# dayae1204/WeCLIP-ViT-CoMer

Measured on AMD Instinct MI355X. Metric: images/sec (train fwd+bwd) ViT-B/16 512x512 VOC, higher is better.
Workload: dtype f16 MFMA operands / f32 accumulate, f32 residual+softmax+LN, PAR f32 arithmetic on 16-bit fixed-point affinities (precision=fast); 1 GPU; WeCLIP VOC full train step (the reference's model: frozen CLIP ViT-B/16 + adapters + decoder + GradCAM/affinity/PAR pseudo-labels), batch 16/GPU at 512x512, K=2 classes/image (BASELINE configs[2] without the ViT-CoMer inserts, for which the reference has no code); global_batch=16, parallelism=dp1

## Files before the change

### include/weclip_hip.h

```cpp
#ifndef WECLIP_HIP_H
#define WECLIP_HIP_H
#include <stdint.h>
#ifdef __cplusplus
extern "C" {
#endif

int wc_version(void);
const char* wc_last_error(void);
int wc_device_count(void);
int wc_device_arch(int dev, char* buf, int buflen);

void wc_prof_enable(int stride);
void wc_prof_tag(const char* tag);
int wc_prof_report(char* buf, int cap);

int wc_par_affinity(const float* img, float* aff, int B, int H, int W,
                    const int* h_dilations, int n_dil, void* stream);
int wc_par_iterate(const float* aff, const float* masks_in, float* masks_out, int B, int C,
                   int H, int W, const int* h_dilations, int n_dil, void* stream);
int wc_par_forward(const float* img, const float* masks, float* out, float* tmp, float* aff_ws,
                   int B, int C, int H, int W, const int* h_dilations, int n_dil, int num_iter,
                   int group, void* stream);
int wc_par_forward_h(const float* img, const float* masks, float* out, float* tmp, float* aff_ws,
                   int B, int C, int H, int W, const int* h_dilations, int n_dil, int num_iter,
                   int group, void* stream);
int wc_par_labels(const float* masks, const int64_t* valid_key, const int* nch, int64_t* labels,
                  int B, int C, int H, int W, void* stream);

int wc_bilinear_resize(const float* src, float* dst, int planes, int Hs, int Ws, int Hd, int Wd,
                       int align_corners, void* stream);
int wc_bilinear_resize_bwd(const float* gdst, float* gsrc, float* tmp, int planes, int Hs, int Ws, int Hd,
                           int Wd, int align_corners, void* stream);

int wc_seg_loss_fwd(const float* seg, const int64_t* label, float* part, float* sums, int B, int nc, int h, int w,
                    int H, int W, int ignore, void* stream);

int wc_seg_loss_fwd_bwd(const float* seg, const int64_t* label, float* cnt, float* part, float* sums, float* tmp, float* grad,
                        int B, int nc, int h, int w, int H, int W, int ignore, void* stream);

int wc_ce_loss_fwd_bwd(const float* seg, const int64_t* label, float* part, float* sums, float* tmp, float* grad, int B, int nc,
                       int h, int w, int H, int W, int ignore, void* stream);

int wc_aff_loss_fwd(const float* attn_pred, const int64_t* cam_label, float* part, float* sums, int B, int h,
                    int w, int H, int W, int radius, int ignore, void* stream);
int wc_aff_loss_bwd(const int64_t* cam_label, const float* coef, float* dap, int B, int h, int w, int H, int W,
                    int radius, int ignore, void* stream);

int wc_gemm_f16(const void* A0, const void* A1, const void* A2, const void* W0, const void* W1,
                const void* W2, int nseg, int M, int N, int K, long lda, long ldw, int batch,
                long sA, long sW, long sC, const float* bias, const float* resid, long ldr, long sR,
                float* C32,
                void* C16, void* C16lo, long ldc, int act, int round16, float scale,
                int scale_cols, float* P32, const float* aux, const int* rowmap, int rpg,
                long ldaux, const void* auxh, const float* cscale, long sCS, void* stream);

int wc_gemm_f16_grouped(const void* A0, const void* A1, const void* A2, const void* W0, const void* W1,
                        const void* W2, int nseg, int M, int N, int K, long lda, long ldw, int batch,
                        long sA, long sW, long sC, const float* bias, const float* resid, long ldr, long sR,
                        float* C32, void* C16, void* C16lo, long ldc, int act, int round16, float scale,
                        int scale_cols, float* P32, const float* aux, const int* rowmap, int rpg,
                        long ldaux, const void* auxh, const float* cscale, long sCS, int zdiv, long sA2, long sW2,
                        long sC2, long sB2, long sX2, void* stream);

int wc_gemm_row_supported(int M, int N, int K);
int wc_gemm_row_f16(const void* A, long lda, const void* W, long ldw, int M, int N, int K, const float* bias,
                    const float* cscale, int act, const float* aux, const void* auxh, long ldaux, const float* resid, long ldr,
                    float* C32, void* C16, float* P32, long ldc, long ldc16, const float* ln_g0, const float* ln_b0, void* ln_o0,
                    const float* ln_g1, const float* ln_b1, void* ln_o1, float eps, void* stream);

int wc_gemm_row_f16_grouped(const void* A, long lda, const void* W, long ldw, int M, int N, int K, const float* bias, int act,
                            const void* auxh, long ldaux, float* C32, void* C16, long ldc, long ldc16, int groups, long gA,
                            long gW, long gB, long gC, long gX, void* stream);

int wc_gemm_plan(int M, int N, int K, int nseg, int batch);
int wc_gemm_log_report(char* buf, int cap);
int wc_sum_slices(const float* part, float* out, int nslices, long n, float alpha, void* stream);

int wc_sum_slices_wb(const float* part, float* out_w, float* out_b, int nslices, int rows, int cols,
                     float alpha, void* stream);
int wc_sum_slices_wb_grouped(const float* part, float* out_w, float* out_b, int nslices, int rows, int cols,
                             float alpha, int groups, long gW, long gB, void* stream);
int wc_sum_slices_wb_multi(const int64_t* jobs, int count, void* stream);

int wc_gemm_km_f16(const void* dY, long lda, const void* X, long ldx, const void* zeros, int M, int N, int K,
                   int x_rpg, int x_gs, int x_off, int mslice, int bias, float* part, void* stream);
int wc_gemm_km_f16_grouped(const void* dY, long lda, const void* X, long ldx, const void* zeros, int M, int N, int K,
                           int x_rpg, int x_gs, int x_off, int mslice, int bias, float* part, int groups, long gA,
                           long gX, void* stream);
int wc_gemm_km_f16_multi(const int64_t* jobs, int count, const void* zeros, void* stream);
int wc_gemm_km_multi_plan(const int64_t* jobs, int count, int cus, int* launch, int* first, int* pos, int* grids,
                          int* forms, int max_launches, int* nlaunches);
int wc_gemm_km_multi_locate(const int64_t* jobs, int count, int cus, int l, int wg, int* out);
int wc_split_f16(const float* x, void* hi, void* lo, long n, void* stream);

int wc_convert_weights(const int64_t* table, int count, int blocks_per_tensor, void* stream);

int wc_adamw_multi(const int64_t* table, int count, double lr, double beta1, double beta2, double eps,
                   double weight_decay, double bias_correction1, double bias_correction2, int blocks_per_tensor,
                   void* stream);

int wc_layernorm(const float* x, long ldx, const float* w, const float* b, float eps, float* y32,
                 void* y16, void* y16lo, long rows, int D, void* stream);

int wc_attn_fwd(const void* qkv, void* out, float* out32, float* lse, int B, int L, int H, int DH,
                void* stream);
int wc_attn_mean(const void* qkv, const float* lse, float* mean, int B, int L, int H, int DH,
                 void* stream);

int wc_patchify(const float* img, void* hi, void* lo, int B, int H, int W, int P, void* stream);
int wc_cls_rows(float* x, const float* cls, const float* pos0, int B, int L, int E, void* stream);

int wc_cam_head(const float* x2, const float* lnw, const float* lnb, const float* proj,
                const float* text, const int* text_idx, const int* n_text, const int* pair_img,
                const int* pair_cls, float logit_scale, float* partial, float* probs, float* df,
                int B, int P, int L, int E, int Ed, int Tmax, void* stream);
int wc_lnpost_bwd(const float* df, const float* x2, const float* lnw, float gs, const int* pair_img,
                  float* d32, void* dhi, void* dlo, int P, int L, int E, void* stream);
int wc_ln2_bwd_add(const float* da2, const float* dx2, const float* x1, const float* lnw, float gs,
                   const int* pair_img, void* g16, int P, int L, int E, void* stream);
int wc_attn_bwd_colsum(const void* qkv, const void* dO, const float* o32, const float* lse,
                       const int* pair_img, float* delta, float* u, float* dS0, float* P0, float* c,
                       int P, int L, int H, int DH, void* stream);
int wc_rowvec_matmul(const float* c, const float* W, float* out, float* ws, int P, int N, int E, float scale,
                     void* stream);
int wc_cam_map(const float* a32, const float* w, const int* pair_img, float* cam, int P, int L, int E,
               void* stream);

int wc_aff_weight(const float* const* h_maps, int nmaps, const float* wgt, const float* seg, float* W,
                  int B, int L, void* stream);
int wc_aff_seg_weights(const float* const* h_maps, int nmaps, const float* seg, float* diff, float* wgt,
                       int B, int L, void* stream);
int wc_matvec(const float* W, const float* X, const float* sin, const float* sout, const float* add,
              float* out, int B, int hw, int K, int transpose, int recip, float alpha, void* stream);
int wc_aff_fused_supported(int hw);
int wc_aff_weight_c1(const float* const* h_maps, int nmaps, const float* wgt, const float* seg, float* W, float* c1,
                     float* ws, int B, int L, void* stream);
int wc_aff_sinkhorn_step(const float* W, const float* c, float* r, float* c_next, float* ws, int B, int hw, int last,
                         void* stream);
int wc_aff_tsym_apply(const float* W, const float* r, const float* c, const float* X, float* out, float* y1, float* ws,
                      int B, int hw, int K, void* stream);
int wc_tsym(const float* W, const float* r, const float* c, float* T, int B, int hw, void* stream);
int wc_box_mask(const float* cam, const int* pair_img, const int* pair_slot, float* V, float* mask_out,
                int* boxes, int* nbox, int maxbox, int P, int h, int w, int K, double thr, void* stream);
int wc_cam_upsample(const float* R, const int* nk, float* stats, float* cams, int B, int h, int w, int K,
                    int C, int H, int W, void* stream);

int wc_attn_bwd(const void* qkv, const void* dO, const float* o32, const float* lse, void* qt, void* kt,
                void* dot, float* delta, void* dqkv_hi, void* dqkv_lo, int B, int L, int Lp, int H, int DH,
                void* stream);
int wc_transpose_f16(const void* src, int src_f32, long ld, long sSrc, void* hi, void* lo, long ldo,
                     long oR, int batch, int R, int C, float scale, void* stream);
int wc_colsum(const void* src, int src_f32, long ld, float* part, float* out, long R, int C, float alpha,
              int round16, void* stream);
int wc_layernorm_bwd(const float* dy, const float* x, const float* w, const float* add, float eps,
                     float* dx32, void* dx16, float out_scale, float* part, float* dgb, float alpha,
                     long rows, int D, void* stream);
int wc_layernorm_bwd_h(const void* dy16, const float* x, const float* w, const float* add, float eps,
                       float* dx32, void* dx16, float out_scale, float* part, float* dgb, float alpha,
                       long rows, int D, void* stream);
int wc_layernorm_bwd2_h(const void* dya16, const float* wa, const void* dyb16, const float* wb, const float* x,
                        const float* add, float eps, float* dx32, void* dx16, float out_scale, float* part, float* dgba,
                        float* dgbb, float alpha, long rows, int D, void* stream);
int wc_sigmoid_gram_bwd(const float* dAP, const float* AP, void* hi, void* lo, int B, int n, int ldo,
                        float scale, void* stream);
int wc_colscale_split(const float* x, const float* cs, float* out32, void* hi, void* lo, long rows, int C,
                      int rows_per_batch, float alpha, void* stream);

int wc_msda_fwd(const float* value, const int* h_shapes, int n_levels, const float* loc, const float* attn,
                float* out, int N, int Lq, int M, int D, int P, void* stream);
int wc_msda_fwd_h(const void* value, int value_is_f16, const int* h_shapes, int n_levels, const float* loc,
                  const float* attn, float* out, void* out16, int N, int Lq, int M, int D, int P, void* stream);
int wc_msda_bwd(const float* value, const int* h_shapes, int n_levels, const float* loc, const float* attn,
                const float* gout, float* gvalue, float* gloc, float* gattn, void* gmax, void* ws, int N, int Lq, int M,
                int D, int P, void* stream);
int wc_msda_bwd_h(const void* value, int value_is_f16, const int* h_shapes, int n_levels, const float* loc,
                  const float* attn, const void* gout, int gout_is_f16, float* gvalue, void* gvalue16, float* gloc,
                  float* gattn, void* gmax, void* ws, int N, int Lq, int M, int D, int P, void* stream);

int wc_dwconv_fwd(const float* x, const float* w, const float* bias, float* y, int N, int C, int H, int W, int k,
                  void* stream);
int wc_dwconv_bwd(const float* x, const float* w, const float* dy, float* dx, float* dw, float* db, float* part,
                  int N, int C, int H, int W, int k, void* stream);

int wc_im2col3x3(const float* x, void* cols_hi, void* cols_lo, int N, int H, int W, int C, int stride, int Kp,
                 void* stream);
int wc_col2im3x3(const float* dcols, float* dx, int N, int H, int W, int C, int stride, int Kp, void* stream);
int wc_groupnorm_relu_fwd(const float* x, const float* gamma, const float* beta, float* y, float* stats, float* part,
                          int N, int HW, int C, int G, float eps, void* stream);
int wc_groupnorm_relu_bwd(const float* x, const float* y, const float* dy, const float* stats, const float* gamma,
                          float* dx, float* dgamma, float* dbeta, float* gpart, float* cpart, float* gsum, int N,
                          int HW, int C, int G, void* stream);

int wc_scale_flip_pair(const float* src, float* dst, int C, int Hs, int Ws, int Hd, int Wd, float scale_y,
                       float scale_x, void* stream);
int wc_flip_avg(const float* segs, float* out, int C, int Hs, int Ws, int Hd, int Wd, float weight, int accumulate,
                void* stream);
int wc_resize_argmax(const float* seg, long* pred, int C, int Hs, int Ws, int Hd, int Wd, void* stream);
int wc_confusion_hist(const long* label_true, const long* label_pred, long* hist, int* flag, long n, int nc,
                      void* stream);

int wc_msda_fused_supported(int n_levels, int M, int D, int P);
int wc_msda_fwd_f(const void* value, int value_is_f16, const int* h_shapes, int n_levels, const float* ow, int ld,
                  const float* bias_off, const float* bias_aw, const float* ref, int nl_ref, float* loc, float* attn,
                  float* out, void* out16, int N, int Lq, int M, int D, int P, void* stream);
int wc_msda_bwd_f(const void* value, int value_is_f16, const int* h_shapes, int n_levels, const float* loc,
                  const float* attn, const void* gout, int gout_is_f16, float* gvalue, void* gvalue16, void* dow16,
                  int ld, void* gmax, void* ws, int N, int Lq, int M, int D, int P, void* stream);

int wc_mrfp_dwconv_fwd(const float* x, const float* w3, const float* b3, const float* w5, const float* b5, float* y,
                       void* g16, const int* h_shapes, int n_levels, int N, int C, void* stream);
int wc_mrfp_dwconv_parts(const int* h_shapes, int n_levels, int N, int C, long* n_parts);
int wc_mrfp_dwconv_bwd(const void* dy, int dy_is_f16, const float* x, const float* w3, const float* w5, float* dx32, void* dx16,
                       float* dw3, float* db3, float* dw5, float* db5, float* part, float alpha, const int* h_shapes,
                       int n_levels, int N, int C, void* stream);
int wc_msda_prep_fwd(const float* ow, const float* bias_off, const float* bias_aw, const float* ref, float* loc, float* attn,
                     const int* h_shapes, int n_levels, int N, int Lq, int M, int P, int ld, int nl_ref, void* stream);
int wc_msda_prep_bwd(const float* gloc, const float* gattn, const float* attn, float* dow32, void* dow16,
                     const int* h_shapes, int n_levels, int N, int Lq, int M, int P, int ld, void* stream);
int wc_rows_copy_f16(const void* src, int src_is_f32, void* dst, int B, int R, int C, long ld_src, long s_src,
                     long ld_dst, long s_dst, void* stream);
int wc_rows_add_f32(const float* src, float* dst, int B, int R, int C, long ld_src, long s_src, long s_dst, float alpha,
                    void* stream);

int wc_cti_gate_grads(const float* G, const float* gs, const float* gamma, const float* Wop, const float* bop, float* dWop,
                      float* dbop, float* dgamma, int C, int K, void* stream);

int wc_augment_workspace_ints(int B, int crop, long* n_ints);
int wc_augment_normalize(const void* src_u8, const void* params, float* dst, int* coeff_ws, int B, int Hs, int Ws, int crop,
                         const float* mean3, const float* std3, void* stream);
int wc_augment_normalize_ragged(const void* src_u8, long src_bytes, const int64_t* offsets, const int* sizes, const void* params,
                                float* dst, int* coeff_ws, int B, int crop, const float* mean3, const float* std3, void* stream);
int wc_normalize_u8(const void* src_u8, const void* lab_u8, float* dst, int64_t* dst_label, int H, int W, const double* mean3,
                    const double* std3, void* stream);

int wc_seg_augment_workspace_ints(int B, int crop, int canvas_max, int n_cand, long* n_ints);
int wc_seg_augment(const void* src_u8, const void* lab_u8, const void* params, const int* cand, float* dst, int64_t* dst_label,
                   int* sel, int* img_box, int* ws, int B, int Hs, int Ws, int crop, int canvas_max, int n_cand, int ignore_index,
                   const float* mean3, const float* std3, void* stream);
int wc_seg_augment_ragged(const void* src_u8, const void* lab_u8, long src_bytes, const int64_t* offsets, const int* sizes,
                          const void* params, const int* cand, float* dst, int64_t* dst_label, int* sel, int* img_box, int* ws,
                          int B, int crop, int canvas_max, int n_cand, int ignore_index, const float* mean3, const float* std3,
                          void* stream);
int wc_seg_crop_select(const void* lab_u8, const void* params, const int* cand, int* sel, int* img_box, int* ws, int B, int Hs,
                       int Ws, int crop, int canvas_max, int n_cand, int ignore_index, void* stream);
int wc_hsv8_convert(const void* src_u8, void* dst_u8, long n, int inverse, void* stream);

int wc_dcrf_unary_prob(const float* probs, float* unary, int C, int H, int W, void* stream);
int wc_dcrf_unary_label(const int64_t* labels, float* unary, int C, int H, int W, float gt_prob, void* stream);
int wc_dcrf_unary_logits(const float* logits, float* unary, int C, int h, int w, int H, int W, void* stream);
int wc_dcrf_workspace_floats(int C, int H, int W, long* n_floats);
int wc_dcrf_inference(const void* img, int img_is_u8, const float* unary, float* Q, void* ws, int C, int H, int W,
                      int iter_max, float pos_w, float pos_xy_std, float bi_w, float bi_xy_std, float bi_rgb_std, void* stream);
int wc_dcrf_message(const void* img, int img_is_u8, const float* Q, float* msg_pos, float* msg_bil, float* S, void* ws,
                    int C, int H, int W, float pos_xy_std, float bi_xy_std, float bi_rgb_std, void* stream);

int wc_energy_workspace_floats(int N, int K, int H, int W, long* n_floats);
int wc_bilateral_filter_batch(const float* images, const float* segs, float* AS, void* ws, int N, int K, int H, int W,
                              float sigma_rgb, float sigma_xy, void* stream);
int wc_dense_energy_fwd(const float* images, const float* segs, const float* rois, const void* unlabel_u8, float* A, float* gate,
                        float* loss, void* ws, int N, int K, int H, int W, float sigma_rgb, float sigma_xy, void* stream);
int wc_dense_energy_bwd(const float* A, const float* rois, const float* grad_out, float* grad_segs, int N, int K, int H, int W,
                        void* stream);

int wc_energy_prep_fwd(const float* img, const float* seg, const int64_t* label, const int* img_box, const float* mean,
                       const float* std, float* images_s, float* P_s, float* rois_s, void* unlabel_u8, int N, int K, int h, int w,
                       int H, int W, int e, void* stream);
int wc_energy_prep_workspace_floats(int N, int K, int h, int W, long* n_floats);
int wc_energy_prep_bwd(const float* A, const float* rois_s, const float* seg, float* grad_seg, void* ws, float coef, int N, int K,
                       int h, int w, int H, int W, int e, void* stream);

int wc_text_embed(const int* tokens, int N, int Lctx, const float* tok_emb, int V, const float* pos, int W, int L,
                  float* x, int* eot, int* bad, void* stream);
int wc_attn_fwd_causal(const void* qkv, void* out, float* out32, float* lse, float* mean, int N, int L, int H, int DH,
                       void* stream);
int wc_text_pool(const float* x, const int* eot, int N, int L, int W, const float* ln_w, const float* ln_b, float eps,
                 const float* proj, int Ed, float* feat, void* stream);
int wc_text_zeroshot(const float* feat, int C, int T, int Ed, float* out, void* stream);

int wc_clip_preprocess_workspace_bytes(int B, int H0, int W0, int h, int w, long* n_bytes);
int wc_clip_preprocess(const void* src_u8, float* dst, float* dst_flip, void* out_u8, void* ws, long ws_bytes, int B, int H0, int W0, int h,
                       int w, const float* mean3, const float* std3, void* stream);
int wc_cam_scale_resize_f16(const float* cam, const int* sizes, const int64_t* offsets, void* out_f16, long out_elems, int P, int gh,
                            int gw, int max_pixels, void* stream);
int wc_cam_resize_f32(const float* cam, const int* sizes, const int64_t* offsets, float* out, long out_elems, int P, int gh, int gw,
                      int max_pixels, void* stream);

int wc_val_pair_hist(const float* seg, const long* cam, const long* gt, long* seg_hist, long* cam_hist, int* flag, int C, int Hs,
                     int Ws, int Hl, int Wl, int nc, void* stream);
int wc_label_match_count(const float* seg, const long* label, long* counts, int B, int C, int Hs, int Ws, int H, int W,
                         void* stream);
int wc_step_pair_hist(const float* seg, const long* label, long* hist, int* flag, int B, int C, int Hs, int Ws, int H, int W,
                      int nc, void* stream);

int wc_eval_finish(const float* seg1, const float* msc, const long* cam, const long* gt, void* pred1_u8, void* predm_u8,
                   void* cmap_rgb, long* hist, long* msc_hist, long* cam_hist, int* flag, int C, int Hs, int Ws, int Hl, int Wl,
                   int nc, void* stream);
int wc_label_finish(const long* pred, const long* gt, void* out_u8, void* cmap_rgb, long* hist, int* flag, int H, int W, int nc,
                    void* stream);

int wc_aff_propagate_workspace_floats(int B, int n, int C, int with_bkg, long* n_floats);
int wc_aff_propagate(const float* aff, const float* mask, const float* cams, const float* cls, float* out, void* ws, int B, int n,
                     int C, float bkg_score, int with_bkg, void* stream);
int wc_cam_to_label(const float* cam, const float* cls, const int* box, long* label, float* valid_cam, int B, int C, int H, int W,
                    float bkg_score, float high_thre, float low_thre, int ignore_mid, long ignore_index, void* stream);
int wc_box_ignore(const void* label, const int* box, void* out, int B, int H, int W, int is_f32, long ignore_index, void* stream);
int wc_bkg_refine_prep(const float* cams, const int* meta, float* stack, int B, int C, int H, int W, int h2, int w2, int Kmax,
                       float high_thre, float low_thre, void* stream);
int wc_bkg_refine_finish(const float* stack, const int* meta, const int* box, float* out, int B, int H, int W, int h2, int w2,
                         int Kmax, float ignore_index, void* stream);
int wc_box_gather(const float* cams, const float* images, const int* meta, float* cams_out, float* img_out, int G, int B, int C,
                  int H, int W, int hb, int wb, int Kg, void* stream);
int wc_box_scatter(const float* src, const int* meta, float* out, int G, int B, int C, int H, int W, int hb, int wb, int Kg,
                   void* stream);

#ifdef __cplusplus
}
#endif
#endif
```

### weclip-vit-comer_amd/WeCLIP_model/model_attn_aff_voc.py

```python
import os

import numpy as np
import torch
import torch.nn as nn

from .. import cam_pipeline as CP
from ..clip import clip_tool as CT
from ..clip import vit_engine as VE
from ..clip.clip import load as clip_load
from ..head_engine import DecoderFunction, HeadEngine, HeadFunction
from ..pytorch_grad_cam import GradCAM
from .comer import CoMerInteraction
from .Decoder.TransDecoder import DecoderTransformer
from .PAR import PAR, refine_labels
from .segformer_head import SegFormerHead


TEMPLATES = ["a clean origami {}."]


def zeroshot_classifier(classnames, templates, model):
    from ..clip import text_engine
    return text_engine.zeroshot(model, list(classnames), list(templates))


def default_text_features(encoder, fg_name, bg_name):
    import importlib
    from ..clip.tokenizer import BPENotFound, bpe_path
    if encoder.transformer.layers == 0:
        return None
    try:
        names = importlib.import_module(__name__.rsplit(".", 2)[0] + ".clip.clip_text")
        bg, fg = getattr(names, bg_name), getattr(names, fg_name)
        bpe_path()
    except (ImportError, AttributeError, BPENotFound):
        return None
    return zeroshot_classifier(bg, TEMPLATES, encoder), zeroshot_classifier(fg, TEMPLATES, encoder)


def reshape_transform(tensor, height=28, width=28):
    t = tensor.permute(1, 0, 2)[:, 1:, :]
    return t.reshape(t.size(0), height, width, t.size(2)).permute(0, 3, 1, 2)


class WeCLIP(nn.Module):
    cam_threshold = 0.4
    seg_trans_last = 6
    seg_trans_after = 15000
    val_runs_cam = True
    fg_names, bg_names = "new_class_names", "BACKGROUND_CATEGORY"

    def __init__(self, num_classes=None, clip_model=None, embedding_dim=256, in_channels=512,
                 dataset_root_path=None, device="cuda", text_features=None, comer=False):
        super().__init__()
        self.num_classes, self.embedding_dim, self.in_channels = num_classes, embedding_dim, in_channels
        self.encoder, _ = clip_load(clip_model, device=device)
        for name, p in self.encoder.named_parameters():
            p.requires_grad = "11" in name
        self.decoder_fts_fuse = SegFormerHead(in_channels=in_channels, embedding_dim=embedding_dim,
                                              num_classes=num_classes, index=11)
        self.decoder = DecoderTransformer(width=embedding_dim, layers=3, heads=8, output_dim=num_classes)
        if text_features is None:
            text_features = default_text_features(self.encoder, self.fg_names, self.bg_names)
        self.bg_text_features, self.fg_text_features = (None, None) if text_features is None else text_features
        self.target_layers = [self.encoder.visual.transformer.resblocks[-1].ln_1]
        self.grad_cam = GradCAM(model=self.encoder, target_layers=self.target_layers,
                                reshape_transform=reshape_transform)
        self.root_path = os.path.join(dataset_root_path, "SegmentationClassAug") if dataset_root_path else None
        self.cam_bg_thres = 1
        self.encoder.eval()
        self.par = PAR(num_iter=20, dilations=[1, 2, 4, 8, 12, 24])
        self.iter_num = 0
        self.require_all_fts = True
        self.head_impl = os.environ.get("WECLIP_HEAD", "hip")
        self.head_engine = HeadEngine(self.decoder_fts_fuse, self.decoder)
        self.comer = CoMerInteraction(embedding_dim) if comer else None
        self.fork_head = os.environ.get("WECLIP_FORK_HEAD", "1") != "0"
        self.to(device)

    def get_param_groups(self):
        groups = [[], [], [], []]
        groups[3].extend(self.decoder.parameters())
        groups[3].extend(self.decoder_fts_fuse.parameters())
        if self.comer is not None:
            groups[3].extend(self.comer.parameters())
        return groups

    def _labels_for(self, img_names, labels, shape):
        if labels is not None:
            return [list(l) for l in labels], [tuple(shape)] * len(labels)
        if self.root_path is None:
            raise RuntimeError("pass labels=[[class ids]...] or construct WeCLIP with dataset_root_path")
        out, sizes = [], []
        for name in img_names:
            ids, osz = CT.read_image_labels(os.path.join(self.root_path, str(name) + ".png"))
            out.append(ids)
            sizes.append(osz)
        return out, sizes

    def _maps_needed(self, seg_trans):
        n = self.seg_trans_last if seg_trans else 8
        first = 12 - n
        return [i >= first for i in range(11)]

    def encode(self, img, seg_trans, x16=None, want_maps=True):
        need = self._maps_needed(seg_trans) if want_maps else [False] * 11
        return VE.encode_blocks(self.encoder.visual, img, need, x16)

    def forward(self, img, img_names="2007_000032", mode="train", labels=None, plan=None, sizes=None):
        B, _, H, W = img.shape
        h, w = H // 16, W // 16
        self.encoder.eval()
        self.iter_num += 1
        seg_trans = self.iter_num > self.seg_trans_after or mode == "val"
        img = img.cuda().float().contiguous()
        hip_head = self.head_impl == "hip" and self.comer is None
        self._bwd_forked = False
        comer_tokens = self.comer is not None and self.head_impl == "hip" and self.comer.engine_ok(img)
        x16 = VE.X16Stack(self.encoder.visual.transformer.layers - 1) if (hip_head or comer_tokens) else None
        with torch.no_grad():
            want_cam = not (mode == "val" and not self.val_runs_cam)
            xs, maps, _, Lq = self.encode(img, seg_trans, x16, want_maps=want_cam)
        if hip_head:
            drop = self.head_engine.draw_dropout(B, img.device) if self.training else None
            fork = self.fork_head and want_cam and img.is_cuda
            if fork:
                main = torch.cuda.current_stream()
                side = CT.side_stream(img.device)
                self.head_engine.fwd_stream = side
                try:
                    seg, attn_pred = HeadFunction.apply(self.head_engine, x16, B, Lq, h, w, drop, *self.head_engine.params())
                finally:
                    self.head_engine.fwd_stream = None

                def joined_attn_pred():
                    main.wait_stream(side)
                    return attn_pred.detach()

                with torch.no_grad():
                    cam_labels = self.cam_labels(img, xs[-1], maps, joined_attn_pred if seg_trans else None, img_names, labels, mode,
                                                 seg_trans, h, w, plan=plan, sizes=sizes)
                main.wait_stream(side)
                return seg, cam_labels, attn_pred
            seg, attn_pred = HeadFunction.apply(self.head_engine, x16, B, Lq, h, w, drop, *self.head_engine.params())
        else:
            fork = self.fork_head and want_cam and not seg_trans and img.is_cuda and self.head_impl == "hip" and self.training
            if fork:
                main = torch.cuda.current_stream()
                side = CT.side_stream(img.device)
                side.wait_stream(main)
                self._bwd_forked = True
                with torch.cuda.stream(side):
                    seg, attn_pred = self._module_head(img, xs, x16, comer_tokens, B, Lq, h, w)
                with torch.no_grad():
                    cam_labels = self.cam_labels(img, xs[-1], maps, None, img_names, labels, mode, seg_trans, h, w, plan=plan, sizes=sizes)
                main.wait_stream(side)
                return seg, cam_labels, attn_pred
            seg, attn_pred = self._module_head(img, xs, x16, comer_tokens, B, Lq, h, w)
        if mode == "val" and not self.val_runs_cam:
            return seg, None, attn_pred
        with torch.no_grad():
            cam_labels = self.cam_labels(img, xs[-1], maps, attn_pred.detach(), img_names, labels, mode,
                                         seg_trans, h, w, plan=plan, sizes=sizes)
        return seg, cam_labels, attn_pred

    def side_streams(self):
        if not getattr(self, "_bwd_forked", False):
            return []
        return CT.side_streams()

    def _module_head(self, img, xs, x16, comer_tokens, B, Lq, h, w):
        if comer_tokens:
            fts = self.decoder_fts_fuse.dropout(self.comer.forward_tokens(img, x16, Lq, self.decoder_fts_fuse.linears_modulelist,
                                                                          (h, w)))
        elif self.comer is not None:
            used = set(self.comer.stage_blocks)
            toks = [mlp.tokens(r.view(B, Lq, -1)[:, 1:, :]) if i in used else None for i, (mlp, r) in
                    enumerate(zip(self.decoder_fts_fuse.linears_modulelist, xs))]
            fts = self.decoder_fts_fuse.dropout(self.comer(img, toks, (h, w)))
        else:
            fts = self.decoder_fts_fuse.forward_rows(xs, B, Lq, h, w)
        if self.head_impl == "hip":
            rows = fts.permute(0, 2, 3, 1).reshape(B * h * w, fts.shape[1])
            seg, attn_pred = DecoderFunction.apply(self.head_engine, rows, B, h, w, *self.head_engine.dec_params())
        else:
            seg, _ = self.decoder(fts, need_weights=False)
            f = fts.reshape(B, fts.shape[1], h * w)
            attn_pred = torch.sigmoid(f.transpose(2, 1).bmm(f))
        return seg, attn_pred

    def cam_labels(self, img, last_rows, maps, attn_pred, img_names, labels, mode, seg_trans, h, w, plan=None, sizes=None):
        if self.bg_text_features is None or self.fg_text_features is None:
            raise RuntimeError("WeCLIP needs text_features=(bg, fg) (see __init__): pass them, or call "
                               "install_dropin(reference_root=<reference checkout>) before constructing WeCLIP so that "
                               "they are computed from clip.clip_text and the BPE vocabulary")
        B, _, H, W = img.shape
        if isinstance(img_names, str):
            img_names = [img_names]
        dev = img.device
        given = sizes
        if plan is None:
            label_lists, sizes = self._labels_for(img_names, labels, (H, W))
            plan = CT.PairPlan(label_lists, self.fg_text_features.shape[0], self.bg_text_features.shape[0], dev)
        else:
            sizes = [(H, W)] * plan.B
        if given is not None:
            sizes = [tuple(int(v) for v in s) for s in given]
        text_hat = CT.normalised_text(self.fg_text_features, self.bg_text_features, dev)
        R, _, _, _ = CT.batch_refined_cams(self.encoder, last_rows, maps, attn_pred if seg_trans else None,
                                           plan, text_hat, h, w, self.cam_threshold, seg_trans,
                                           self.seg_trans_last)
        C = plan.K + 1
        if mode == "train" or all(tuple(s) == (H, W) for s in sizes):
            cams = CP.upsample_with_bg(R, plan.nk, h, w, H, W, C)
            refined = self.par(img, cams)
            return refine_labels(refined, plan.valid_key, plan.nch)
        out = []
        for i, (oh, ow) in enumerate(sizes):
            cams = CP.upsample_with_bg(R[i:i + 1].contiguous(), plan.nk[i:i + 1].contiguous(), h, w, oh, ow, C)
            refined = self.par(img[i:i + 1], cams)
            out.append(refine_labels(refined, plan.valid_key[i:i + 1].contiguous(),
                                     plan.nch[i:i + 1].contiguous())[0])
        return out
```

### weclip-vit-comer_amd/cam_pipeline.py

```python
import ctypes

import torch

from . import _lib as L
from .ops import F32

I32 = torch.int32


def _map_array(maps):
    arr = (ctypes.c_void_p * len(maps))(*[m.data_ptr() for m in maps])
    return arr


def seg_layer_keep(maps, n_last=6):
    sel = maps[-n_last:]
    B, Lq, _ = sel[0].shape
    hw = Lq - 1
    dev = sel[0].device
    for m in sel:
        L.ptr(m, F32, "attention map")
    diff = torch.empty(B, len(sel), device=dev, dtype=F32)
    wgt = torch.empty(B, len(sel), device=dev, dtype=F32)
    rowsum = torch.empty(B, len(sel), hw, device=dev, dtype=F32)
    L.lib().wc_aff_seg_weights(_map_array(sel), len(sel), L.ptr(rowsum), L.ptr(diff), L.ptr(wgt), B, Lq, L.stream())
    return (wgt > 0).float()


def fused_ok(hw):
    return hw % 4 == 0 and 4 <= hw <= 2048


def _nblk(hw):
    return (hw + 31) // 32


def affinity_weight(maps, seg=None, seg_trans=False, n_last=6, keep=None, return_c1=False):
    sel = maps[-n_last:] if seg_trans else maps[-8:]
    B, Lq, _ = sel[0].shape
    hw = Lq - 1
    dev = sel[0].device
    for m in sel:
        L.ptr(m, F32, "attention map")
    lib = L.lib()
    W = torch.empty(B, hw, hw, device=dev, dtype=F32)

    def weight(wgt, segp):
        if return_c1 and fused_ok(hw):
            c1 = torch.empty(B, hw, device=dev, dtype=F32)
            ws = torch.empty(B * ((hw + 7) // 8) * hw, device=dev, dtype=F32)
            lib.wc_aff_weight_c1(_map_array(sel), len(sel), L.ptr(wgt), L.ptr(segp), L.ptr(W), L.ptr(c1), L.ptr(ws), B, Lq,
                                 L.stream())
            return W, c1
        lib.wc_aff_weight(_map_array(sel), len(sel), L.ptr(wgt), L.ptr(segp), L.ptr(W), B, Lq, L.stream())
        return (W, None) if return_c1 else W

    if not seg_trans:
        wgt = torch.full((B, len(sel)), 1.0 / len(sel), device=dev, dtype=F32)
        return weight(wgt, None)
    seg = seg.detach().float().contiguous()
    if keep is not None:
        keep = keep.to(dev).float()
        wgt = (keep / (keep.sum(1, keepdim=True) + 1e-5)).contiguous()
    else:
        diff = torch.empty(B, len(sel), device=dev, dtype=F32)
        wgt = torch.empty(B, len(sel), device=dev, dtype=F32)
        rowsum = torch.empty(B, len(sel), hw, device=dev, dtype=F32)
        lib.wc_aff_seg_weights(_map_array(sel), len(sel), L.ptr(rowsum), L.ptr(diff), L.ptr(wgt), B, Lq, L.stream())
    return weight(wgt, seg)


def _matvec(W, X, sin=None, sout=None, add=None, transpose=False, recip=False, alpha=1.0):
    B, hw, _ = W.shape
    K = X.shape[-1]
    out = torch.empty(B, hw, K, device=W.device, dtype=F32)
    L.lib().wc_matvec(L.ptr(W, F32), L.ptr(X, F32), L.ptr(sin, F32), L.ptr(sout, F32), L.ptr(add, F32),
                      L.ptr(out), B, hw, K, 1 if transpose else 0, 1 if recip else 0, alpha, L.stream())
    return out


def sinkhorn_scales(W, rounds=3, c1=None):
    B, hw, _ = W.shape
    if fused_ok(hw):
        lib = L.lib()
        ws = torch.empty(B * _nblk(hw) * hw, device=W.device, dtype=F32)
        if c1 is None:
            c1 = _matvec(W, torch.ones(B, hw, 1, device=W.device, dtype=F32), transpose=True, recip=True).view(B, hw)
        c = c1
        for it in range(rounds):
            r = torch.empty(B, hw, device=W.device, dtype=F32)
            last = it == rounds - 1
            cn = None if last else torch.empty(B, hw, device=W.device, dtype=F32)
            lib.wc_aff_sinkhorn_step(L.ptr(W, F32), L.ptr(c, F32), L.ptr(r), L.ptr(cn), L.ptr(ws), B, hw, 1 if last else 0,
                                     L.stream())
            if not last:
                c = cn
        return r, c
    r = torch.ones(B, hw, 1, device=W.device, dtype=F32)
    c = None
    for _ in range(rounds):
        c = _matvec(W, r, transpose=True, recip=True)
        r = _matvec(W, c, transpose=False, recip=True)
    return r.view(B, hw), c.view(B, hw)


def tsym_apply(W, r, c, X):
    B, hw, _ = W.shape
    K = X.shape[-1]
    if fused_ok(hw):
        out = torch.empty(B, hw, K, device=W.device, dtype=F32)
        for k0 in range(0, K, 4):
            kn = min(4, K - k0)
            Xs = X if (k0 == 0 and kn == K) else X[:, :, k0:k0 + kn].contiguous()
            os_ = out if (k0 == 0 and kn == K) else torch.empty(B, hw, kn, device=W.device, dtype=F32)
            y1 = torch.empty(B, hw, kn, device=W.device, dtype=F32)
            ws = torch.empty(B * _nblk(hw) * hw * kn, device=W.device, dtype=F32)
            L.lib().wc_aff_tsym_apply(L.ptr(W, F32), L.ptr(r.contiguous(), F32), L.ptr(c.contiguous(), F32), L.ptr(Xs, F32),
                                      L.ptr(os_), L.ptr(y1), L.ptr(ws), B, hw, kn, L.stream())
            if os_ is not out:
                out[:, :, k0:k0 + kn] = os_
        return out
    half = _matvec(W, X, sin=c, sout=r, alpha=0.5)
    return _matvec(W, X, sin=r, sout=c, add=half, transpose=True, alpha=0.5)


def trans_mat(W):
    B, hw, _ = W.shape
    r, c = sinkhorn_scales(W)
    T = torch.empty(B, hw, hw, device=W.device, dtype=F32)
    L.lib().wc_tsym(L.ptr(W, F32), L.ptr(r), L.ptr(c), L.ptr(T), B, hw, L.stream())
    out = torch.empty_like(T)
    for k0 in range(0, hw, 64):
        X = T[:, :, k0:k0 + 64].contiguous()
        out[:, :, k0:k0 + 64] = _matvec(T, X)
    return out


def box_masks(cams, pair_img, pair_slot, B, K, h, w, thr, want_mask=False, want_boxes=False):
    P = cams.shape[0]
    dev = cams.device
    V = torch.zeros(B, h * w, K, device=dev, dtype=F32)
    mask = torch.empty(P, h * w, device=dev, dtype=F32) if want_mask else None
    boxes = torch.zeros(P, 64, 4, device=dev, dtype=I32) if want_boxes else None
    nbox = torch.zeros(P, device=dev, dtype=I32) if want_boxes else None
    L.lib().wc_box_mask(L.ptr(cams, F32, "cams"), L.ptr(pair_img, I32), L.ptr(pair_slot, I32), L.ptr(V),
                        L.ptr(mask), L.ptr(boxes), L.ptr(nbox), 64, P, h, w, K, float(thr), L.stream())
    return V, mask, boxes, nbox


def refine(W, cams, pair_img, pair_slot, K, h, w, thr, c1=None):
    B = W.shape[0]
    r, c = sinkhorn_scales(W, c1=c1)
    V, _, _, _ = box_masks(cams, pair_img, pair_slot, B, K, h, w, thr)
    return tsym_apply(W, r, c, tsym_apply(W, r, c, V))


def upsample_with_bg(R, nk, h, w, H, Wd, C=None):
    B, hw, K = R.shape
    C = K + 1 if C is None else C
    stats = torch.empty(B, K, 2, device=R.device, dtype=F32)
    cams = torch.empty(B, C, H, Wd, device=R.device, dtype=F32)
    L.lib().wc_cam_upsample(L.ptr(R, F32), L.ptr(nk, I32), L.ptr(stats), L.ptr(cams), B, h, w, K, C, H, Wd,
                            L.stream())
    return cams
```

### weclip-vit-comer_amd/clip/clip_tool.py

```python
import os

import numpy as np
import torch

from .. import cam_pipeline as CP
from ..gradcam_engine import last_layer_forward
from . import vit_engine as VE

I32 = torch.int32


class ClipOutputTarget:
    def __init__(self, category):
        self.category = category

    def __call__(self, model_output):
        return model_output[self.category] if model_output.dim() == 1 else model_output[:, self.category]


def generate_clip_fts(image, model, require_all_fts=True):
    if image.dim() == 3:
        image = image.unsqueeze(0)
    h, w = image.shape[-2:]
    return model.encode_image(image.cuda(), h, w, require_all_fts=require_all_fts)


def compute_trans_mat(attn_weight):
    from .. import torch_ops
    return torch.ops.weclip.trans_mat(attn_weight.detach().float().contiguous()[None].cuda())[0]


def read_image_labels(img_path):
    from PIL import Image
    arr = np.asarray(Image.open(img_path))
    ids = (np.unique(arr) - 1).tolist()
    ids = [int(i) for i in ids if i not in (255, 254)]
    return ids, arr.shape[:2]


class PairPlan:
    PAD_P = 8

    def __init__(self, label_lists, n_fg, n_bg, device, pad=False):
        self.pad = bool(pad)
        self.n_fg, self.n_bg, self.device = n_fg, n_bg, torch.device(device)
        host, vk = self._host_arrays(label_lists)
        cuda = self.device.type == "cuda"
        self._host = host.pin_memory() if cuda else host
        self._host_vk = vk.pin_memory() if cuda else vk
        self._dev_all = self._host.to(self.device, non_blocking=True)
        self.valid_key = self._host_vk.to(self.device, non_blocking=True)
        views, off = [], 0
        for n in self._part_len:
            views.append(self._dev_all[off:off + n])
            off += n
        self.pair_img, self.pair_cls, self.pair_slot, text_idx, self.n_text, self.nk, self.nch = views
        self.text_idx = text_idx.view(self.P, self.Tmax)

    @staticmethod
    def signature(label_lists, pad=False):
        P, K = sum(len(l) for l in label_lists), max(len(l) for l in label_lists)
        if pad:
            P, K = -(-P // PairPlan.PAD_P) * PairPlan.PAD_P, max(2, K + (K & 1))
        return len(label_lists), P, K

    def _host_arrays(self, label_lists):
        self.label_lists = [list(map(int, l)) for l in label_lists]
        if any(len(l) == 0 for l in self.label_lists):
            raise RuntimeError("every image needs at least one foreground class id")
        self.B, P_sig, self.K = self.signature(self.label_lists, self.pad)
        self.Tmax = self.K + self.n_bg
        pi, pc, ps, ti, nt = [], [], [], [], []
        for i, ids in enumerate(self.label_lists):
            rows = ids + [self.n_fg + r for r in range(self.n_bg)]
            for j in range(len(ids)):
                pi.append(i); pc.append(j); ps.append(j)
                ti.append(rows + [0] * (self.Tmax - len(rows)))
                nt.append(len(rows))
        self.P_real = len(pi)
        for _ in range(P_sig - len(pi)):
            pi.append(pi[0]); pc.append(pc[0]); ps.append(-1)
            ti.append(list(ti[0]))
            nt.append(nt[0])
        nk = [len(l) for l in self.label_lists]
        flat_ti = [v for row in ti for v in row]
        parts = [pi, pc, ps, flat_ti, nt, nk, [k + 1 for k in nk]]
        self._part_len = [len(p) for p in parts]
        self.P = len(pi)
        host = torch.tensor([v for part in parts for v in part], dtype=I32)
        vk = torch.zeros(self.B, self.K + 1, dtype=torch.int64)
        for i, ids in enumerate(self.label_lists):
            vk[i, 1:1 + len(ids)] = torch.tensor(ids) + 1
        return host, vk

    def update(self, label_lists):
        if self.signature(label_lists, self.pad) != (self.B, self.P, self.K):
            raise RuntimeError(f"PairPlan.update: signature {self.signature(label_lists, self.pad)} != {(self.B, self.P, self.K)}")
        host, vk = self._host_arrays(label_lists)
        if self.device.type != "cuda":
            self._dev_all.copy_(host)
            self.valid_key.copy_(vk)
            return self
        if not hasattr(self, "_ring"):
            self._ring = [(self._host, self._host_vk, None), (self._host.clone().pin_memory(), self._host_vk.clone().pin_memory(), None)]
            self._slot = 0
        self._slot ^= 1
        h, v, ev = self._ring[self._slot]
        if ev is not None:
            ev.synchronize()
        h.copy_(host)
        v.copy_(vk)
        self._dev_all.copy_(h, non_blocking=True)
        self.valid_key.copy_(v, non_blocking=True)
        ev = ev or torch.cuda.Event()
        ev.record()
        self._ring[self._slot] = (h, v, ev)
        return self


def normalised_text(fg_text, bg_text, device):
    t = torch.cat([fg_text.detach().float(), bg_text.detach().float()], 0).to(device)
    return (t / t.norm(dim=1, keepdim=True)).contiguous()


def batch_refined_cams(clip_model, last_rows, maps11, seg_attn, plan, text_hat, h, w, thr,
                       seg_trans, n_last, keep=None):
    B, Lq = plan.B, h * w + 1
    st = last_layer_forward(clip_model, last_rows, B, Lq)
    maps = list(maps11) + [st.mean]
    need = maps[-n_last:] if seg_trans else maps[-8:]
    if any(m is None for m in need):
        raise RuntimeError("attention maps needed by the affinity were not computed")
    if callable(seg_attn):
        if seg_trans:
            cams, probs, _ = st.grad_cam(text_hat, plan.text_idx, plan.n_text, plan.pair_img, plan.pair_cls, plan.Tmax)
            W, c1 = CP.affinity_weight(maps, seg_attn(), seg_trans, n_last, keep=keep, return_c1=True)
            R = CP.refine(W, cams, plan.pair_img, plan.pair_slot, plan.K, h, w, thr, c1=c1)
            return R, cams, probs, st
        seg_attn = None
    cams, probs, _ = st.grad_cam(text_hat, plan.text_idx, plan.n_text, plan.pair_img, plan.pair_cls, plan.Tmax)
    W, c1 = CP.affinity_weight(maps, seg_attn, seg_trans, n_last, keep=keep, return_c1=True)
    R = CP.refine(W, cams, plan.pair_img, plan.pair_slot, plan.K, h, w, thr, c1=c1)
    return R, cams, probs, st


_SIDE = {}


def side_stream(dev):
    key = (dev.type, dev.index if dev.index is not None else torch.cuda.current_device())
    if key not in _SIDE:
        _SIDE[key] = torch.cuda.Stream(device=dev)
    return _SIDE[key]


def side_streams():
    return list(_SIDE.values())


def _single(img_path, image, image_features, attn_weight_list, seg_attn, bg_text_features, fg_text_features,
            cam, mode, require_seg_trans, thr, n_last, labels=None):
    if labels is None:
        ids, (oh, ow) = read_image_labels(img_path)
    else:
        ids, (oh, ow) = list(labels), image.shape[-2:]
    H, W = image.shape[-2:]
    h, w = H // 16, W // 16
    dev = image_features.device
    rows, N, Lq = VE.to_rows(image_features)
    plan = PairPlan([ids], fg_text_features.shape[0], bg_text_features.shape[0], dev)
    text_hat = normalised_text(fg_text_features, bg_text_features, dev)
    maps = [m[None].float().contiguous() for m in attn_weight_list]
    seg = seg_attn.reshape(1, h * w, h * w) if seg_attn is not None else None
    R, _, _, _ = batch_refined_cams(cam.model, rows, maps, seg, plan, text_hat, h, w, thr, require_seg_trans, n_last)
    refined = [R[0, :, k].reshape(h, w) for k in range(len(ids))]
    return (refined, ids, W, H) if mode == "train" else (refined, ids, ow, oh)


def perform_single_voc_cam(img_path, image, image_features, attn_weight_list, seg_attn, bg_text_features,
                           fg_text_features, cam, mode="train", require_seg_trans=False, labels=None):
    return _single(img_path, image, image_features, attn_weight_list, seg_attn, bg_text_features,
                   fg_text_features, cam, mode, require_seg_trans, 0.4, 6, labels)


def perform_single_coco_cam(img_path, image, image_features, attn_weight_list, seg_attn, bg_text_features,
                            fg_text_features, cam, mode="train", require_all_fts=True, require_seg_trans=False,
                            labels=None):
    return _single(img_path, image, image_features, attn_weight_list, seg_attn, bg_text_features,
                   fg_text_features, cam, mode, require_seg_trans, 0.7, 10, labels)


def generate_cam_label(cam_refined_list, keys, w, h):
    R = torch.stack([c.reshape(-1) for c in cam_refined_list], dim=1)[None].float().contiguous().cuda()
    hh, ww = cam_refined_list[0].shape
    nk = torch.tensor([len(cam_refined_list)], dtype=I32, device="cuda")
    cams = CP.upsample_with_bg(R, nk, hh, ww, h, w)
    return {"keys": np.asarray(keys), "refined_cam": cams[0, 1:]}
```

### weclip-vit-comer_amd/clip/vit_engine.py

```python
import torch

from .. import config, ops
from ..ops import F16, F32, Split


class BlockPack:

    def __init__(self, blk, exact=None, pre=None):
        exact = config.exact() if exact is None else exact
        pre = pre or {}
        at = blk.attn
        self.E = at.embed_dim
        self.H = at.num_heads
        self.DH = self.E // self.H
        self.exact = exact
        f = lambda p: p.detach().float().contiguous()
        self.ln1_w, self.ln1_b = f(blk.ln_1.weight), f(blk.ln_1.bias)
        self.ln2_w, self.ln2_b = f(blk.ln_2.weight), f(blk.ln_2.bias)
        self.in_w = pre.get("in_w") or ops.split_f16(at.in_proj_weight, with_lo=exact)
        self.in_b = f(at.in_proj_bias)
        self.out_w = pre.get("out_w") or ops.split_f16(at.out_proj.weight, with_lo=False)
        self.out_b = f(at.out_proj.bias).half().float()
        self.fc_w = pre.get("fc_w") or ops.split_f16(blk.mlp.c_fc.weight, with_lo=exact and blk.fp32_mlp)
        self.fc_b = f(blk.mlp.c_fc.bias)
        self.pj_w = pre.get("pj_w") or ops.split_f16(blk.mlp.c_proj.weight, with_lo=exact and blk.fp32_mlp)
        self.pj_b = f(blk.mlp.c_proj.bias)


class X16Stack(list):

    def __init__(self, n):
        super().__init__()
        self.n, self.big, self.big_lo = n, None, None

    def next_slot(self, M, E, dev, ex):
        if self.big is None:
            self.big = torch.empty(self.n, M, E, device=dev, dtype=F16)
            self.big_lo = torch.empty(self.n, M, E, device=dev, dtype=F16) if ex else None
        i = len(self)
        if i >= self.n or self.big.shape[1:] != (M, E):
            return None
        return Split(self.big[i], self.big_lo[i] if self.big_lo is not None else None)


def run_block(pk, x, B, L, want_mean=True, keep=None, x16_out=None, tag=None, causal=False):
    M, E, H, DH = B * L, pk.E, pk.H, pk.DH
    dev = x.device
    ex = pk.exact
    a32, a = ops.layernorm(x, pk.ln1_w, pk.ln1_b, want32=keep is not None, with_lo=ex)
    if tag:
        ops.KernelTimer.tag(tag)
    qkv = torch.empty(M, 3 * E, device=dev, dtype=F16)
    ops.gemm(a, pk.in_w, M, 3 * E, E, bias=pk.in_b, out16=qkv, scale=ops.q_scale(DH), scale_cols=E)
    o32 = None
    attn = ops.attention_causal if causal else ops.attention
    if keep is not None:
        o16, lse, mean, o32 = attn(qkv, B, L, H, DH, want_mean=want_mean, want_o32=True)
    else:
        o16, lse, mean = attn(qkv, B, L, H, DH, want_mean=want_mean)
    x1 = torch.empty(M, E, device=dev, dtype=F32)
    ops.gemm(o16, pk.out_w, M, E, E, bias=pk.out_b, resid=x, out32=x1, round16=True)
    if tag:
        ops.KernelTimer.tag(None)
    _, a2 = ops.layernorm(x1, pk.ln2_w, pk.ln2_b, with_lo=ex)
    z = Split(torch.empty(M, 4 * E, device=dev, dtype=F16),
              torch.empty(M, 4 * E, device=dev, dtype=F16) if ex else None)
    u32 = torch.empty(M, 4 * E, device=dev, dtype=F32) if keep is not None else None
    ops.gemm(a2, pk.fc_w, M, 4 * E, E, bias=pk.fc_b, out16=z.hi, out16lo=z.lo, act=1, pre32=u32)
    x2 = torch.empty(M, E, device=dev, dtype=F32)
    x2h = None
    if x16_out is not None:
        exo = ex or bool(int(config.head_lo) & 32)
        nxt = x16_out.next_slot(M, E, dev, exo) if isinstance(x16_out, X16Stack) else None
        x2h = nxt or Split(torch.empty(M, E, device=dev, dtype=F16), torch.empty(M, E, device=dev, dtype=F16) if exo else None)
        x16_out.append(x2h)
    ops.gemm(z, pk.pj_w, M, E, 4 * E, bias=pk.pj_b, resid=x1, out32=x2,
             out16=x2h.hi if x2h else None, out16lo=x2h.lo if x2h else None)
    if keep is not None:
        keep.update(a32=a32, qkv=qkv, o32=o32, lse=lse, x1=x1, u32=u32)
    return x2, mean


def encode_blocks(vis, img, need, x16=None):
    rows, B, Lq = vis.embed(img)
    xs, maps = [], []
    for i in range(vis.transformer.layers - 1):
        rows, m = run_block(vis.transformer.resblocks[i].pack(), rows, B, Lq, want_mean=need[i], x16_out=x16, tag=b"@vit_attn")
        xs.append(rows)
        maps.append(m)
    return xs, maps, B, Lq


def to_rows(x_lne):
    Lq, N, E = x_lne.shape
    return x_lne.detach().float().permute(1, 0, 2).contiguous().view(N * Lq, E), N, Lq


def from_rows(x, N, Lq):
    return x.view(N, Lq, -1).permute(1, 0, 2)
```

### weclip-vit-comer_amd/csrc/affinity.hip

```cpp
#include "common.h"
#include "resample.h"

#define MAXK 4

struct MapPtrs {
    const float* p[12];
};

__global__ __launch_bounds__(256) void aff_weight_kernel(MapPtrs maps, int nmaps, const float* __restrict__ wgt,
                                                          const float* __restrict__ seg, float* __restrict__ W,
                                                          int L) {
    const int hw = L - 1;
    const int j = blockIdx.x * 256 + threadIdx.x, i = blockIdx.y, b = blockIdx.z;
    if (j >= hw) return;
    const long src = (long)b * L * L + (long)(i + 1) * L + (j + 1);
    float v[12];
#pragma unroll
    for (int l = 0; l < 12; ++l) v[l] = l < nmaps ? maps.p[l][src] : 0.f;
    float s = 0.f;
#pragma unroll
    for (int l = 0; l < 12; ++l)
        if (l < nmaps) s = fmaf(wgt[b * nmaps + l], v[l], s);
    const long dst = ((long)b * hw + i) * hw + j;
    if (seg) s *= seg[dst];
    W[dst] = s;
}

__global__ __launch_bounds__(256) void aff_rowsum_kernel(MapPtrs maps, int nmaps, float* __restrict__ rowsum, int L) {
    __shared__ float red[16];
    const int hw = L - 1, i = blockIdx.x, l = blockIdx.y, b = blockIdx.z;
    const float* row = maps.p[l] + (long)b * L * L + (long)(i + 1) * L + 1;
    float s = 0.f;
    for (int j = threadIdx.x; j < hw; j += 256) s += row[j];
    s = block_sum(s, red);
    if (threadIdx.x == 0) rowsum[((long)b * nmaps + l) * hw + i] = s;
}

__global__ __launch_bounds__(64) void aff_keep_kernel(const float* __restrict__ rowsum, float* __restrict__ diff,
                                                       float* __restrict__ wgt, int nmaps, int hw) {
    __shared__ float A[12];
    const int b = blockIdx.x, lane = threadIdx.x;
    for (int l = 0; l < nmaps; ++l) {
        const float* rs = rowsum + ((long)b * nmaps + l) * hw;
        float s = 0.f;
        for (int i = lane; i < hw; i += 64) s += rs[i];
        s = wave_sum(s);
        if (lane == 0) A[l] = s;
    }
    __syncthreads();
    if (lane != 0) return;
    float m = 0.f;
    for (int l = 0; l < nmaps; ++l) m += A[l];
    m /= nmaps;
    float n = 0.f;
    for (int l = 0; l < nmaps; ++l) n += (A[l] >= m) ? 1.f : 0.f;
    for (int l = 0; l < nmaps; ++l) {
        diff[b * nmaps + l] = -A[l];
        wgt[b * nmaps + l] = ((A[l] >= m) ? 1.f : 0.f) / (n + 1e-5f);
    }
}

#define MVC_SLICES 16
__global__ __launch_bounds__(64 * MVC_SLICES) void matvec_cols_kernel(const float* __restrict__ W, const float* __restrict__ X,
                                                           const float* __restrict__ sin, const float* __restrict__ sout,
                                                           const float* __restrict__ add, float* __restrict__ out,
                                                           int hw, int K, int k0, int recip, float alpha) {
    __shared__ float red[MVC_SLICES][64][MAXK];
    constexpr int NS = MVC_SLICES;
    const int lane = threadIdx.x & 63, wv = threadIdx.x >> 6;
    const int j = blockIdx.x * 64 + lane, b = blockIdx.y;
    const int kn = (K - k0 < MAXK) ? K - k0 : MAXK;
    float acc[MAXK] = {0.f, 0.f, 0.f, 0.f};
    if (j < hw) {
        const float* Wb = W + (long)b * hw * hw + j;
        int i = wv;
        for (; i + 7 * NS < hw; i += 8 * NS) {
            float wr[8];
#pragma unroll
            for (int u = 0; u < 8; ++u)
                wr[u] = Wb[(long)(i + NS * u) * hw] * (sin ? sin[(long)b * hw + i + NS * u] : 1.f);
#pragma unroll
            for (int u = 0; u < 8; ++u) {
                const float* xr = X + ((long)b * hw + i + NS * u) * K + k0;
#pragma unroll
                for (int k = 0; k < MAXK; ++k)
                    if (k < kn) acc[k] = fmaf(wr[u], xr[k], acc[k]);
            }
        }
        for (; i < hw; i += NS) {
            const float wv_ = Wb[(long)i * hw] * (sin ? sin[(long)b * hw + i] : 1.f);
            const float* xr = X + ((long)b * hw + i) * K + k0;
#pragma unroll
            for (int k = 0; k < MAXK; ++k)
                if (k < kn) acc[k] = fmaf(wv_, xr[k], acc[k]);
        }
    }
#pragma unroll
    for (int k = 0; k < MAXK; ++k) red[wv][lane][k] = acc[k];
    __syncthreads();
    if (wv == 0 && j < hw) {
        for (int k = 0; k < kn; ++k) {
            float v = 0.f;
#pragma unroll
            for (int q = 0; q < MVC_SLICES; ++q) v += red[q][lane][k];
            const long o = ((long)b * hw + j) * K + k0 + k;
            if (recip) v = 1.0f / v;
            else {
                v *= alpha * (sout ? sout[(long)b * hw + j] : 1.f);
                if (add) v += add[o];
            }
            out[o] = v;
        }
    }
}

__global__ __launch_bounds__(256) void matvec_rows_kernel(const float* __restrict__ W, const float* __restrict__ X,
                                                           const float* __restrict__ sin, const float* __restrict__ sout,
                                                           const float* __restrict__ add, float* __restrict__ out,
                                                           int hw, int K, int k0, int recip, float alpha) {
    const int lane = threadIdx.x & 63;
    const int i = blockIdx.x * 4 + (threadIdx.x >> 6), b = blockIdx.y;
    if (i >= hw) return;
    const int kn = (K - k0 < MAXK) ? K - k0 : MAXK;
    float acc[MAXK] = {0.f, 0.f, 0.f, 0.f};
    const float* Wr = W + ((long)b * hw + i) * hw;
    int j = lane;
    for (; j + 192 < hw; j += 256) {
        float wr[4];
#pragma unroll
        for (int u = 0; u < 4; ++u) wr[u] = Wr[j + 64 * u] * (sin ? sin[(long)b * hw + j + 64 * u] : 1.f);
#pragma unroll
        for (int u = 0; u < 4; ++u) {
            const float* xr = X + ((long)b * hw + j + 64 * u) * K + k0;
#pragma unroll
            for (int k = 0; k < MAXK; ++k)
                if (k < kn) acc[k] = fmaf(wr[u], xr[k], acc[k]);
        }
    }
    for (; j < hw; j += 64) {
        const float wv_ = Wr[j] * (sin ? sin[(long)b * hw + j] : 1.f);
        const float* xr = X + ((long)b * hw + j) * K + k0;
#pragma unroll
        for (int k = 0; k < MAXK; ++k)
            if (k < kn) acc[k] = fmaf(wv_, xr[k], acc[k]);
    }
#pragma unroll
    for (int k = 0; k < MAXK; ++k) acc[k] = wave_sum(acc[k]);
    if (lane == 0)
        for (int k = 0; k < kn; ++k) {
            float v = acc[k];
            const long o = ((long)b * hw + i) * K + k0 + k;
            if (recip) v = 1.0f / v;
            else {
                v *= alpha * (sout ? sout[(long)b * hw + i] : 1.f);
                if (add) v += add[o];
            }
            out[o] = v;
        }
}

#define AF_RPB 32
#define AF_RPBW 8
#define AF_RG 4
#define AF_MAXCH 2

__global__ __launch_bounds__(256) void aff_weight_colpart_kernel(MapPtrs maps, int nmaps, const float* __restrict__ wgt,
                                                                  const float* __restrict__ seg, float* __restrict__ W,
                                                                  float* __restrict__ colpart, int L) {
    const int hw = L - 1, blk = blockIdx.x, b = blockIdx.y, nblk = gridDim.x;
    const int i0 = blk * AF_RPBW, i1 = min(i0 + AF_RPBW, hw);
    float wl[12];
#pragma unroll
    for (int l = 0; l < 12; ++l) wl[l] = l < nmaps ? wgt[b * nmaps + l] : 0.f;
    for (int j = threadIdx.x; j < hw; j += 256) {
        float sacc[AF_RPBW];
#pragma unroll
        for (int r = 0; r < AF_RPBW; ++r) sacc[r] = 0.f;
        const long base = (long)b * L * L + (long)(i0 + 1) * L + (j + 1);
#pragma unroll
        for (int l = 0; l < 12; l += 2) {
            if (l >= nmaps) break;
            float v0[AF_RPBW], v1[AF_RPBW];
            const bool two = l + 1 < nmaps;
#pragma unroll
            for (int r = 0; r < AF_RPBW; ++r) {
                const long src = base + (long)(i0 + r < i1 ? r : 0) * L;
                v0[r] = maps.p[l][src];
                v1[r] = two ? maps.p[l + 1][src] : 0.f;
            }
#pragma unroll
            for (int r = 0; r < AF_RPBW; ++r) {
                sacc[r] = fmaf(wl[l], v0[r], sacc[r]);
                if (two) sacc[r] = fmaf(wl[l + 1], v1[r], sacc[r]);
            }
        }
        float cs = 0.f;
        float sg[AF_RPBW];
        if (seg) {
#pragma unroll
            for (int r = 0; r < AF_RPBW; ++r) sg[r] = seg[((long)b * hw + min(i0 + r, i1 - 1)) * hw + j];
        }
#pragma unroll
        for (int r = 0; r < AF_RPBW; ++r) {
            if (i0 + r >= i1) break;
            const long dst = ((long)b * hw + i0 + r) * hw + j;
            float v = sacc[r];
            if (seg) v *= sg[r];
            W[dst] = v;
            cs += v;
        }
        colpart[((long)b * nblk + blk) * hw + j] = cs;
    }
}

template <int MODE, int K>
__global__ __launch_bounds__(256) void aff_sweep_kernel(const float* __restrict__ W, const float* __restrict__ c,
                                                         const float* __restrict__ rin, const float* __restrict__ X,
                                                         float* __restrict__ rout, float* __restrict__ y1,
                                                         float* __restrict__ colpart, int hw) {
    __shared__ float red[2][4][AF_RG][K];
    const int blk = blockIdx.x, b = blockIdx.y, nblk = gridDim.x;
    const int tid = threadIdx.x, lane = tid & 63, wave = tid >> 6;
    const int i0 = blk * AF_RPB, i1 = min(i0 + AF_RPB, hw);
    const float* Wb = W + (long)b * hw * hw;
    const float* cb = c + (long)b * hw;
    const int nch = (hw + 1023) / 1024;
    float cx[AF_MAXCH][4][K];
    float ca[AF_MAXCH][4][K];
    bool okc[AF_MAXCH];
#pragma unroll
    for (int ch = 0; ch < AF_MAXCH; ++ch) {
        const int j = ch * 1024 + tid * 4;
        okc[ch] = ch < nch && j < hw;
#pragma unroll
        for (int q = 0; q < 4; ++q)
#pragma unroll
            for (int k = 0; k < K; ++k) {
                ca[ch][q][k] = 0.f;
                const int jc = okc[ch] ? j + q : 0;
                float v = cb[jc];
                if (MODE == 2) v *= X[((long)b * hw + jc) * K + k];
                cx[ch][q][k] = v * (okc[ch] ? 1.f : 0.f);
            }
    }
    int buf = 0;
    for (int ig = i0; ig < i1; ig += AF_RG, buf ^= 1) {
        float4 w[AF_RG][AF_MAXCH];
#pragma unroll
        for (int r = 0; r < AF_RG; ++r)
#pragma unroll
            for (int ch = 0; ch < AF_MAXCH; ++ch) {
                const bool ok = okc[ch] && ig + r < i1;
                const float4 t = *reinterpret_cast<const float4*>(Wb + (long)min(ig + r, i1 - 1) * hw + (okc[ch] ? ch * 1024 + tid * 4 : 0));
                const float mk = ok ? 1.f : 0.f;
                w[r][ch] = make_float4(t.x * mk, t.y * mk, t.z * mk, t.w * mk);
            }
        float rix[AF_RG], xix[AF_RG][K];
        if (MODE == 2) {
#pragma unroll
            for (int r = 0; r < AF_RG; ++r) {
                const long i = (long)b * hw + min(ig + r, i1 - 1);
                rix[r] = rin[i];
#pragma unroll
                for (int k = 0; k < K; ++k) xix[r][k] = X[i * K + k];
            }
        }
        float p[AF_RG][K];
#pragma unroll
        for (int r = 0; r < AF_RG; ++r)
#pragma unroll
            for (int k = 0; k < K; ++k) {
                float a = 0.f;
#pragma unroll
                for (int ch = 0; ch < AF_MAXCH; ++ch)
                    a += w[r][ch].x * cx[ch][0][k] + w[r][ch].y * cx[ch][1][k] + w[r][ch].z * cx[ch][2][k] + w[r][ch].w * cx[ch][3][k];
                p[r][k] = wave_sum(a);
            }
        if (lane == 0) {
#pragma unroll
            for (int r = 0; r < AF_RG; ++r)
#pragma unroll
                for (int k = 0; k < K; ++k) red[buf][wave][r][k] = p[r][k];
        }
        __syncthreads();
#pragma unroll
        for (int r = 0; r < AF_RG; ++r) {
            const int i = ig + r;
            if (i >= i1) continue;
            float rv[K];
#pragma unroll
            for (int k = 0; k < K; ++k) {
                const float dot = red[buf][0][r][k] + red[buf][1][r][k] + red[buf][2][r][k] + red[buf][3][r][k];
                if (MODE == 2) {
                    const float ri = rix[r];
                    if (tid == 0) y1[((long)b * hw + i) * K + k] = ri * dot;
                    rv[k] = ri * xix[r][k];
                } else {
                    rv[k] = 1.0f / dot;
                    if (tid == 0) rout[(long)b * hw + i] = rv[k];
                }
            }
            if (MODE != 1) {
#pragma unroll
                for (int ch = 0; ch < AF_MAXCH; ++ch)
#pragma unroll
                    for (int k = 0; k < K; ++k) {
                        ca[ch][0][k] = fmaf(w[r][ch].x, rv[k], ca[ch][0][k]);
                        ca[ch][1][k] = fmaf(w[r][ch].y, rv[k], ca[ch][1][k]);
                        ca[ch][2][k] = fmaf(w[r][ch].z, rv[k], ca[ch][2][k]);
                        ca[ch][3][k] = fmaf(w[r][ch].w, rv[k], ca[ch][3][k]);
                    }
            }
        }
    }
    if (MODE != 1) {
#pragma unroll
        for (int ch = 0; ch < AF_MAXCH; ++ch) {
            if (!okc[ch]) continue;
            const int j = ch * 1024 + tid * 4;
#pragma unroll
            for (int q = 0; q < 4; ++q)
#pragma unroll
                for (int k = 0; k < K; ++k) colpart[(((long)b * nblk + blk) * hw + j + q) * K + k] = ca[ch][q][k];
        }
    }
}

__global__ __launch_bounds__(256) void aff_colreduce_kernel(const float* __restrict__ colpart, const float* __restrict__ y1,
                                                             const float* __restrict__ c, float* __restrict__ out, int hw,
                                                             int K, int nblk, int mode) {
    const int e = blockIdx.x * 256 + threadIdx.x, b = blockIdx.y;
    if (e >= hw * K) return;
    const float* cp = colpart + (long)b * nblk * hw * K + e;
    const long st = (long)hw * K;
    float s = 0.f;
    int blk = 0;
    for (; blk + 8 <= nblk; blk += 8) {
        float v[8];
#pragma unroll
        for (int u = 0; u < 8; ++u) v[u] = cp[(blk + u) * st];
        s += ((v[0] + v[1]) + (v[2] + v[3])) + ((v[4] + v[5]) + (v[6] + v[7]));
    }
    for (; blk < nblk; ++blk) s += cp[blk * st];
    if (mode == 0) out[(long)b * hw + e] = 1.0f / s;
    else out[(long)b * hw * K + e] = 0.5f * (y1[(long)b * hw * K + e] + c[(long)b * hw + e / K] * s);
}

__global__ __launch_bounds__(256) void tsym_kernel(const float* __restrict__ W, const float* __restrict__ r,
                                                    const float* __restrict__ c, float* __restrict__ T, int hw) {
    const int j = blockIdx.x * 256 + threadIdx.x, i = blockIdx.y, b = blockIdx.z;
    if (j >= hw) return;
    const float* Wb = W + (long)b * hw * hw;
    const float* rb = r + (long)b * hw;
    const float* cb = c + (long)b * hw;
    T[((long)b * hw + i) * hw + j] = 0.5f * (rb[i] * Wb[(long)i * hw + j] * cb[j] + cb[i] * Wb[(long)j * hw + i] * rb[j]);
}

__global__ __launch_bounds__(256) void box_mask_kernel(const float* __restrict__ cam, const int* __restrict__ pair_img,
                                                        const int* __restrict__ pair_slot, float* __restrict__ V,
                                                        float* __restrict__ mask_out, int* __restrict__ boxes,
                                                        int* __restrict__ nbox, int maxbox, int h, int w, int K,
                                                        double thr) {
    extern __shared__ int smi[];
    const int hw = h * w, p = blockIdx.x, tid = threadIdx.x;
    int* lab = smi;
    int* xmin = lab + hw;
    int* xmax = xmin + hw;
    int* ymin = xmax + hw;
    int* ymax = ymin + hw;
    int* roots = ymax + hw;
    int* misc = roots + hw;
    const float* cp = cam + (long)p * hw;
    if (tid == 0) { misc[0] = 0; misc[2] = 0; }
    __syncthreads();
    int mx = 0;
    for (int i = tid; i < hw; i += 256) {
        const int u = (int)(unsigned char)(cp[i] * 255.0f);
        mx = u > mx ? u : mx;
    }
    atomicMax(&misc[0], mx);
    __syncthreads();
    const int theta = (int)(thr * (double)misc[0]);
    for (int i = tid; i < hw; i += 256) {
        const int u = (int)(unsigned char)(cp[i] * 255.0f);
        lab[i] = (u > theta) ? i : -1;
        xmin[i] = w; xmax[i] = -1; ymin[i] = h; ymax[i] = -1;
    }
    __syncthreads();
    for (int it = 0; it < hw + 2; ++it) {
        if (tid == 0) misc[1] = 0;
        __syncthreads();
        int changed = 0;
        for (int i = tid; i < hw; i += 256) {
            int l = lab[i];
            if (l < 0) continue;
            const int y = i / w, x = i - y * w;
            int best = l;
            for (int dy = -1; dy <= 1; ++dy)
                for (int dx = -1; dx <= 1; ++dx) {
                    const int yy = y + dy, xx = x + dx;
                    if (yy < 0 || yy >= h || xx < 0 || xx >= w) continue;
                    const int nl = lab[yy * w + xx];
                    if (nl >= 0 && nl < best) best = nl;
                }
            if (best < l) { lab[i] = best; changed = 1; }
        }
        if (changed) misc[1] = 1;
        __syncthreads();
        if (misc[1] == 0) break;
        for (int i = tid; i < hw; i += 256) {
            const int l = lab[i];
            if (l >= 0) {
                const int ll = lab[l];
                if (ll < l) lab[i] = ll;
            }
        }
        __syncthreads();
    }
    for (int i = tid; i < hw; i += 256) {
        int l = lab[i];
        if (l < 0) continue;
        while (lab[l] != l) l = lab[l];
        const int y = i / w, x = i - y * w;
        atomicMin(&xmin[l], x); atomicMax(&xmax[l], x);
        atomicMin(&ymin[l], y); atomicMax(&ymax[l], y);
    }
    __syncthreads();
    for (int i = tid; i < hw; i += 256)
        if (lab[i] == i) roots[atomicAdd(&misc[2], 1)] = i;
    __syncthreads();
    const int nroot = misc[2];
    if (boxes) {
        if (tid == 0) nbox[p] = nroot;
        for (int k = tid; k < nroot && k < maxbox; k += 256) {
            const int r = roots[k];
            int* bx = boxes + ((long)p * maxbox + k) * 4;
            bx[0] = xmin[r]; bx[1] = ymin[r];
            bx[2] = (xmax[r] + 1 < w - 1) ? xmax[r] + 1 : w - 1;
            bx[3] = (ymax[r] + 1 < h - 1) ? ymax[r] + 1 : h - 1;
        }
    }
    const int img = pair_img[p], slot = pair_slot[p];
    for (int i = tid; i < hw; i += 256) {
        const int y = i / w, x = i - y * w;
        int inside = 0;
        for (int k = 0; k < nroot && !inside; ++k) {
            const int r = roots[k];
            const int x0 = xmin[r], y0 = ymin[r];
            int x1 = xmax[r] + 1, y1 = ymax[r] + 1;
            x1 = x1 < w - 1 ? x1 : w - 1;
            y1 = y1 < h - 1 ? y1 : h - 1;
            inside = (x >= x0 && x < x1 && y >= y0 && y < y1);
        }
        if (mask_out) mask_out[(long)p * hw + i] = inside ? 1.f : 0.f;
        if (slot >= 0) V[((long)img * hw + i) * K + slot] = inside ? cp[i] : 0.f;
    }
}

__global__ __launch_bounds__(256) void refined_minmax_kernel(const float* __restrict__ R, float* __restrict__ stats,
                                                              int hw, int K) {
    __shared__ float red[16];
    const int k = blockIdx.x, b = blockIdx.y;
    float mn = INFINITY, mx = -INFINITY;
    for (int i = threadIdx.x; i < hw; i += 256) {
        const float v = R[((long)b * hw + i) * K + k];
        mn = fminf(mn, v);
        mx = fmaxf(mx, v);
    }
    mn = block_min(mn, red);
    mx = block_max(mx, red);
    if (threadIdx.x == 0) {
        stats[((long)b * K + k) * 2] = mn;
        stats[((long)b * K + k) * 2 + 1] = mx - mn;
    }
}

__global__ __launch_bounds__(256) void cam_upsample_kernel(const float* __restrict__ R, const float* __restrict__ stats,
                                                            const int* __restrict__ nk, float* __restrict__ cams,
                                                            int h, int w, int K, int C, int H, int W, float sy, float sx) {
    const int x = blockIdx.x * 64 + (threadIdx.x & 63), y = blockIdx.y * 4 + (threadIdx.x >> 6), b = blockIdx.z;
    if (x >= W || y >= H) return;
    int y0, y1, x0, x1;
    float ly, lx;
    wc_bil_src(y, h, sy, y0, y1, ly);
    wc_bil_src(x, w, sx, x0, x1, lx);
    const long HW = (long)H * W;
    const int n = nk[b];
    float best = -INFINITY;
    const float* Rb = R + (long)b * h * w * K;
    for (int k = 0; k < n; ++k) {
        const float mn = stats[((long)b * K + k) * 2], den = 1e-7f + stats[((long)b * K + k) * 2 + 1];
        const float v00 = (Rb[((long)y0 * w + x0) * K + k] - mn) / den, v01 = (Rb[((long)y0 * w + x1) * K + k] - mn) / den;
        const float v10 = (Rb[((long)y1 * w + x0) * K + k] - mn) / den, v11 = (Rb[((long)y1 * w + x1) * K + k] - mn) / den;
        const float v = wc_lerp4(v00, v01, v10, v11, ly, lx);
        cams[((long)b * C + 1 + k) * HW + (long)y * W + x] = v;
        best = fmaxf(best, v);
    }
    for (int k = n; k < C - 1; ++k) cams[((long)b * C + 1 + k) * HW + (long)y * W + x] = 0.f;
    cams[(long)b * C * HW + (long)y * W + x] = 1.0f - best;
}

extern "C" int wc_aff_weight(const float* const* h_maps, int nmaps, const float* wgt, const float* seg, float* W,
                             int B, int L, void* stream) {
    WC_CHECK_ARG(h_maps && nmaps >= 1 && nmaps <= 12 && wgt && W && B > 0 && L > 1, "wc_aff_weight: bad argument");
    MapPtrs mp;
    for (int i = 0; i < 12; ++i) mp.p[i] = i < nmaps ? h_maps[i] : nullptr;
    const int hw = L - 1;
    hipLaunchKernelGGL(aff_weight_kernel, dim3(wc_cdiv(hw, 256), hw, B), dim3(256), 0, (hipStream_t)stream, mp, nmaps,
                       wgt, seg, W, L);
    WC_LAUNCH_CHECK("aff_weight_kernel");
    return WC_OK;
}

extern "C" int wc_aff_seg_weights(const float* const* h_maps, int nmaps, float* rowsum, float* diff, float* wgt,
                                  int B, int L, void* stream) {
    WC_CHECK_ARG(h_maps && nmaps >= 1 && nmaps <= 12 && rowsum && diff && wgt && B > 0 && L > 1,
                 "wc_aff_seg_weights: bad argument");
    MapPtrs mp;
    for (int i = 0; i < 12; ++i) mp.p[i] = i < nmaps ? h_maps[i] : nullptr;
    hipStream_t st = (hipStream_t)stream;
    hipLaunchKernelGGL(aff_rowsum_kernel, dim3(L - 1, nmaps, B), dim3(256), 0, st, mp, nmaps, rowsum, L);
    WC_LAUNCH_CHECK("aff_rowsum_kernel");
    hipLaunchKernelGGL(aff_keep_kernel, dim3(B), dim3(64), 0, st, rowsum, diff, wgt, nmaps, L - 1);
    WC_LAUNCH_CHECK("aff_keep_kernel");
    return WC_OK;
}

extern "C" int wc_matvec(const float* W, const float* X, const float* sin, const float* sout, const float* add,
                         float* out, int B, int hw, int K, int transpose, int recip, float alpha, void* stream) {
    WC_CHECK_ARG(W && X && out && B > 0 && hw > 0 && K > 0 && B <= 65535, "wc_matvec: bad argument");
    WC_CHECK_ARG(out != X && out != sin, "wc_matvec: out must not alias an input vector");
    hipStream_t st = (hipStream_t)stream;
    for (int k0 = 0; k0 < K; k0 += MAXK) {
        if (transpose)
            hipLaunchKernelGGL(matvec_cols_kernel, dim3(wc_cdiv(hw, 64), B), dim3(64 * MVC_SLICES), 0, st, W, X, sin, sout, add,
                               out, hw, K, k0, recip, alpha);
        else
            hipLaunchKernelGGL(matvec_rows_kernel, dim3(wc_cdiv(hw, 4), B), dim3(256), 0, st, W, X, sin, sout, add,
                               out, hw, K, k0, recip, alpha);
        WC_LAUNCH_CHECK("matvec kernel");
    }
    return WC_OK;
}

static bool aff_fused_ok(int hw) { return hw % 4 == 0 && hw <= 1024 * AF_MAXCH && hw >= 4; }

extern "C" int wc_aff_fused_supported(int hw) { return aff_fused_ok(hw) ? 1 : 0; }

extern "C" int wc_aff_weight_c1(const float* const* h_maps, int nmaps, const float* wgt, const float* seg, float* W, float* c1,
                                float* ws, int B, int L, void* stream) {
    WC_CHECK_ARG(h_maps && nmaps >= 1 && nmaps <= 12 && wgt && W && c1 && ws && B > 0 && B <= 65535 && L > 1 && aff_fused_ok(L - 1),
                 "wc_aff_weight_c1: bad argument");
    MapPtrs mp;
    for (int i = 0; i < 12; ++i) mp.p[i] = i < nmaps ? h_maps[i] : nullptr;
    const int hw = L - 1, nblk = wc_cdiv(hw, AF_RPBW);
    hipStream_t st = (hipStream_t)stream;
    const int pr = wc_prof_begin(stream);
    hipLaunchKernelGGL(aff_weight_colpart_kernel, dim3(nblk, B), dim3(256), 0, st, mp, nmaps, wgt, seg, W, ws, L);
    wc_prof_end(pr, "aff_weight_colpart_kernel", (double)B * hw * hw * 4.0 * (nmaps + 1 + (seg ? 1 : 0)), stream);
    WC_LAUNCH_CHECK("aff_weight_colpart_kernel");
    hipLaunchKernelGGL(aff_colreduce_kernel, dim3(wc_cdiv(hw, 256), B), dim3(256), 0, st, ws, nullptr, nullptr, c1, hw, 1, nblk, 0);
    WC_LAUNCH_CHECK("aff_colreduce_kernel");
    return WC_OK;
}

extern "C" int wc_aff_sinkhorn_step(const float* W, const float* c, float* r, float* c_next, float* ws, int B, int hw,
                                    int last, void* stream) {
    WC_CHECK_ARG(W && c && r && ws && (last || c_next) && B > 0 && B <= 65535 && aff_fused_ok(hw), "wc_aff_sinkhorn_step: bad argument");
    const int nblk = wc_cdiv(hw, AF_RPB);
    hipStream_t st = (hipStream_t)stream;
    const int pr = wc_prof_begin(stream);
    if (last) hipLaunchKernelGGL((aff_sweep_kernel<1, 1>), dim3(nblk, B), dim3(256), 0, st, W, c, nullptr, nullptr, r, nullptr, ws, hw);
    else hipLaunchKernelGGL((aff_sweep_kernel<0, 1>), dim3(nblk, B), dim3(256), 0, st, W, c, nullptr, nullptr, r, nullptr, ws, hw);
    wc_prof_end(pr, "aff_sweep_kernel", (double)B * hw * hw * 4.0 * (last ? 1 : 2), stream);
    WC_LAUNCH_CHECK("aff_sweep_kernel");
    if (!last) {
        hipLaunchKernelGGL(aff_colreduce_kernel, dim3(wc_cdiv(hw, 256), B), dim3(256), 0, st, ws, nullptr, nullptr, c_next, hw, 1, nblk, 0);
        WC_LAUNCH_CHECK("aff_colreduce_kernel");
    }
    return WC_OK;
}

extern "C" int wc_aff_tsym_apply(const float* W, const float* r, const float* c, const float* X, float* out, float* y1,
                                 float* ws, int B, int hw, int K, void* stream) {
    WC_CHECK_ARG(W && r && c && X && out && y1 && ws && out != X && B > 0 && B <= 65535 && K >= 1 && K <= 4 && aff_fused_ok(hw),
                 "wc_aff_tsym_apply: bad argument (K <= 4)");
    const int nblk = wc_cdiv(hw, AF_RPB);
    hipStream_t st = (hipStream_t)stream;
    dim3 grid(nblk, B);
    const int pr = wc_prof_begin(stream);
    switch (K) {
        case 1: hipLaunchKernelGGL((aff_sweep_kernel<2, 1>), grid, dim3(256), 0, st, W, c, r, X, nullptr, y1, ws, hw); break;
        case 2: hipLaunchKernelGGL((aff_sweep_kernel<2, 2>), grid, dim3(256), 0, st, W, c, r, X, nullptr, y1, ws, hw); break;
        case 3: hipLaunchKernelGGL((aff_sweep_kernel<2, 3>), grid, dim3(256), 0, st, W, c, r, X, nullptr, y1, ws, hw); break;
        default: hipLaunchKernelGGL((aff_sweep_kernel<2, 4>), grid, dim3(256), 0, st, W, c, r, X, nullptr, y1, ws, hw); break;
    }
    wc_prof_end(pr, "aff_sweep_kernel", (double)B * hw * hw * 4.0 * 2, stream);
    WC_LAUNCH_CHECK("aff_sweep_kernel");
    hipLaunchKernelGGL(aff_colreduce_kernel, dim3(wc_cdiv(hw * K, 256), B), dim3(256), 0, st, ws, y1, c, out, hw, K, nblk, 1);
    WC_LAUNCH_CHECK("aff_colreduce_kernel");
    return WC_OK;
}

extern "C" int wc_tsym(const float* W, const float* r, const float* c, float* T, int B, int hw, void* stream) {
    WC_CHECK_ARG(W && r && c && T && B > 0 && hw > 0, "wc_tsym: bad argument");
    hipLaunchKernelGGL(tsym_kernel, dim3(wc_cdiv(hw, 256), hw, B), dim3(256), 0, (hipStream_t)stream, W, r, c, T, hw);
    WC_LAUNCH_CHECK("tsym_kernel");
    return WC_OK;
}

extern "C" int wc_box_mask(const float* cam, const int* pair_img, const int* pair_slot, float* V, float* mask_out,
                           int* boxes, int* nbox, int maxbox, int P, int h, int w, int K, double thr, void* stream) {
    WC_CHECK_ARG(cam && pair_img && pair_slot && V && P > 0 && h > 0 && w > 0 && K > 0, "wc_box_mask: bad argument");
    WC_CHECK_ARG(!boxes || (nbox && maxbox > 0), "wc_box_mask: boxes needs nbox and maxbox");
    const size_t sm = ((size_t)6 * h * w + 4) * sizeof(int);
    WC_CHECK_ARG(sm <= 160 * 1024, "wc_box_mask: CAM grid too large (h*w <= 6800)");
    hipLaunchKernelGGL(box_mask_kernel, dim3(P), dim3(256), sm, (hipStream_t)stream, cam, pair_img, pair_slot, V,
                       mask_out, boxes, nbox, maxbox, h, w, K, thr);
    WC_LAUNCH_CHECK("box_mask_kernel");
    return WC_OK;
}

extern "C" int wc_cam_upsample(const float* R, const int* nk, float* stats, float* cams, int B, int h, int w, int K,
                               int C, int H, int W, void* stream) {
    WC_CHECK_ARG(R && nk && stats && cams && B > 0 && h > 0 && w > 0 && K > 0 && C >= 2 && C <= K + 1 && H > 0 && W > 0,
                 "wc_cam_upsample: bad argument");
    hipStream_t st = (hipStream_t)stream;
    hipLaunchKernelGGL(refined_minmax_kernel, dim3(K, B), dim3(256), 0, st, R, stats, h * w, K);
    WC_LAUNCH_CHECK("refined_minmax_kernel");
    hipLaunchKernelGGL(cam_upsample_kernel, dim3(wc_cdiv(W, 64), wc_cdiv(H, 4), B), dim3(256), 0, st, R, stats, nk,
                       cams, h, w, K, C, H, W, (float)h / H, (float)w / W);
    WC_LAUNCH_CHECK("cam_upsample_kernel");
    return WC_OK;
}
```

### weclip-vit-comer_amd/csrc/attention.hip

```cpp
#include "common.h"
#include <stdlib.h>

typedef _Float16 f16x8 __attribute__((ext_vector_type(8)));
typedef _Float16 f16x4 __attribute__((ext_vector_type(4)));
typedef _Float16 f16x2 __attribute__((ext_vector_type(2)));
typedef float f32x16 __attribute__((ext_vector_type(16)));

#define NEG_BIG (-1.0e30f)

template <int DH, int NT>
__device__ __forceinline__ void attn_row_body(const __half* __restrict__ qkv, __half* __restrict__ out,
                                              float* __restrict__ out32, float* __restrict__ lse, int L, int H,
                                              int E, int q, int h, int b, float* lds) {
    constexpr int NCH = DH / 8;
    constexpr int NPT = NT / NCH;
    float* sc = lds;
    float* red = lds + ((L + 3) & ~3);
    float (*part)[DH] = reinterpret_cast<float (*)[DH]>(red + 16);
    const int tid = threadIdx.x;
    const long ldq = 3L * E;
    const __half* base = qkv + (long)b * L * ldq + (long)h * DH;
    f16x8 qv[NCH];
#pragma unroll
    for (int c = 0; c < NCH; ++c) qv[c] = *reinterpret_cast<const f16x8*>(base + (long)q * ldq + c * 8);
    float mx = NEG_BIG;
    for (int key = tid; key < L; key += NT) {
        const __half* kr = base + E + (long)key * ldq;
        float s = 0.f;
#pragma unroll
        for (int c = 0; c < NCH; ++c) {
            const f16x8 kv = *reinterpret_cast<const f16x8*>(kr + c * 8);
#pragma unroll
            for (int j = 0; j < 8; ++j) s = fmaf((float)qv[c][j], (float)kv[j], s);
        }
        sc[key] = s;
        mx = fmaxf(mx, s);
    }
    mx = block_max(mx, red);
    float sum = 0.f;
    for (int key = tid; key < L; key += NT) {
        const float pr = __builtin_amdgcn_exp2f(sc[key] - mx);
        sum += pr;
        sc[key] = (float)(_Float16)pr;
    }
    sum = block_sum(sum, red);
    const int ch = tid % NCH, pt = tid / NCH;
    float o[8];
#pragma unroll
    for (int j = 0; j < 8; ++j) o[j] = 0.f;
    const __half* vcol = base + 2 * E + ch * 8;
    int key = pt;
    for (; key + 3 * NPT < L; key += 4 * NPT) {
        f16x8 v[4];
#pragma unroll
        for (int u = 0; u < 4; ++u) v[u] = *reinterpret_cast<const f16x8*>(vcol + (long)(key + u * NPT) * ldq);
#pragma unroll
        for (int u = 0; u < 4; ++u) {
            const float pr = sc[key + u * NPT];
#pragma unroll
            for (int j = 0; j < 8; ++j) o[j] = fmaf(pr, (float)v[u][j], o[j]);
        }
    }
    for (; key < L; key += NPT) {
        const f16x8 v = *reinterpret_cast<const f16x8*>(vcol + (long)key * ldq);
        const float pr = sc[key];
#pragma unroll
        for (int j = 0; j < 8; ++j) o[j] = fmaf(pr, (float)v[j], o[j]);
    }
#pragma unroll
    for (int j = 0; j < 8; ++j) part[pt][ch * 8 + j] = o[j];
    __syncthreads();
    if (tid < DH) {
        float v = 0.f;
        for (int k = 0; k < NPT; ++k) v += part[k][tid];
        v /= sum;
        const long oi = ((long)b * L + q) * E + (long)h * DH + tid;
        out[oi] = __float2half(v);
        if (out32) out32[oi] = v;
        if (tid == 0) lse[((long)b * H + h) * L + q] = mx + log2f(sum);
    }
}

#define ATT_EDGE_MAX 8
template <int DH, int NW>
__global__ __launch_bounds__(NW * 64, 4) void attn_fwd_kernel(const __half* __restrict__ qkv,
                                                        __half* __restrict__ out,
                                                        float* __restrict__ out32,
                                                        float* __restrict__ lse, int L, int H,
                                                        int E, int q_origin, int nqb, int Bn, int k_origin) {
    constexpr int NT = NW * 64;
    constexpr int KS = DH / 16;
    constexpr int DT = DH / 32;
    constexpr int KROW = DH * 2 + 16;
    constexpr int VROW = DH * 2;
    constexpr int KBUF = 64 * KROW, VBUF = 64 * VROW;
    constexpr int KCH = DH / 8;
    constexpr int TCH = 64 * KCH;
    constexpr int NKC = (TCH + NT - 1) / NT;
    constexpr int NVC = NKC;
    extern __shared__ __attribute__((aligned(16))) char smem[];

    const int tid = threadIdx.x, lane = tid & 63, wave = tid >> 6;
    const int hh = lane >> 5, l31 = lane & 31;
    const int per_img = nqb * H;
    const int main_blocks = per_img * ((Bn + 7) / 8 * 8);
    if ((int)blockIdx.x >= main_blocks) {
        const int e = blockIdx.x - main_blocks;
        const int hb = e / q_origin;
        attn_row_body<DH, NT>(qkv, out, out32, lse, L, H, E, e - hb * q_origin, hb % H, hb / H, reinterpret_cast<float*>(smem));
        return;
    }
    const int slot = blockIdx.x >> 3;
    const int b = (slot / per_img) * 8 + (blockIdx.x & 7);
    if (b >= Bn) return;
    const int rem = slot - (slot / per_img) * per_img;
    const int h = rem / nqb, qb = rem - h * nqb;
    const int qrow = q_origin + qb * (NW * 32) + wave * 32 + l31;
    const int qr = qrow < L ? qrow : L - 1;
    const long ldq = 3L * E;
    const __half* base = qkv + (long)b * L * ldq + (long)h * DH;

    f16x8 qf[KS];
#pragma unroll
    for (int s = 0; s < KS; ++s)
        qf[s] = *reinterpret_cast<const f16x8*>(base + (long)qr * ldq + 16 * s + 8 * hh);

    u32x4 rk[NKC], rv[NVC];
#define VSWZ(key_) (DH == 64 ? ((((key_) >> 1) & 1) << 2) : 0)
    int vaddr[2];
    {
        const int gi = (lane >> 4) & 1, q4 = (lane >> 2) & 3, p4 = lane & 3;
#pragma unroll
        for (int r = 0; r < 2; ++r) {
            const int key = 8 * r + 4 * hh + q4;
            vaddr[r] = key * VROW + (((2 * gi + (p4 >> 1)) ^ VSWZ(key)) << 4) + 8 * (p4 & 1);
        }
    }
    typedef short s16x4 __attribute__((__vector_size__(4 * sizeof(short))));
    typedef __attribute__((address_space(3))) s16x4* tr_ptr;
#undef GLOAD
#define GLOAD(t_) \
    { \
        const int t__ = (t_); \
        _Pragma("unroll") \
        for (int i = 0; i < NKC; ++i) { \
            const int c = (NKC * NT == TCH) ? tid + NT * i : (tid + NT * i) % TCH;    \
            int key = k_origin + t__ * 64 + c / KCH; \
            if (key > L - 1) key = L - 1; \
            rk[i] = *reinterpret_cast<const u32x4*>(base + E + (long)key * ldq + (c % KCH) * 8); \
        } \
        _Pragma("unroll") \
        for (int i = 0; i < NVC; ++i) { \
            const int c = (NKC * NT == TCH) ? tid + NT * i : (tid + NT * i) % TCH; \
            int key = k_origin + t__ * 64 + c / KCH; \
            if (key > L - 1) key = L - 1; \
            rv[i] = *reinterpret_cast<const u32x4*>(base + 2 * E + (long)key * ldq + (c % KCH) * 8); \
        } \
    }
#undef LSTORE
#define LSTORE(buf_) \
    { \
        const int buf__ = (buf_); \
        char* kb = smem + buf__ * (KBUF + VBUF); \
        char* vb = kb + KBUF; \
        _Pragma("unroll") \
        for (int i = 0; i < NKC; ++i) { \
            const int c = tid + NT * i; \
            if (c < TCH) *reinterpret_cast<u32x4*>(kb + (c / KCH) * KROW + (c % KCH) * 16) = rk[i]; \
        } \
        _Pragma("unroll") \
        for (int i = 0; i < NVC; ++i) { \
            const int c = tid + NT * i; \
            const int key__ = c / KCH; \
            if (c < TCH) *reinterpret_cast<u32x4*>(vb + key__ * VROW + (((c % KCH) ^ VSWZ(key__)) << 4)) = rv[i]; \
        } \
    }

    f32x16 o[DT];
#pragma unroll
    for (int d = 0; d < DT; ++d)
#pragma unroll
        for (int r = 0; r < 16; ++r) o[d][r] = 0.f;
    float m = NEG_BIG, lsum = 0.f;

    const int nt = (L - k_origin + 63) / 64;
    GLOAD(0);
    LSTORE(0);
    __syncthreads();
    for (int t = 0; t < nt; ++t) {
        const int buf = t & 1;
        if (t + 1 < nt) GLOAD(t + 1);
        const char* kb = smem + buf * (KBUF + VBUF);
        const char* vb = kb + KBUF;
        f32x16 s[2];
#pragma unroll
        for (int r = 0; r < 16; ++r) { s[0][r] = 0.f; s[1][r] = 0.f; }
#pragma unroll
        for (int ks = 0; ks < KS; ++ks) {
            const f16x8 a0 = *reinterpret_cast<const f16x8*>(kb + l31 * KROW + ks * 32 + hh * 16);
            const f16x8 a1 = *reinterpret_cast<const f16x8*>(kb + (32 + l31) * KROW + ks * 32 + hh * 16);
            s[0] = __builtin_amdgcn_mfma_f32_32x32x16_f16(a0, qf[ks], s[0], 0, 0, 0);
            s[1] = __builtin_amdgcn_mfma_f32_32x32x16_f16(a1, qf[ks], s[1], 0, 0, 0);
        }
        if (t == nt - 1) {
#pragma unroll
            for (int ti = 0; ti < 2; ++ti)
#pragma unroll
                for (int r = 0; r < 16; ++r) {
                    const int key = k_origin + t * 64 + ti * 32 + (r & 3) + 8 * (r >> 2) + 4 * hh;
                    if (key >= L) s[ti][r] = NEG_BIG;
                }
        }
        float mx = s[0][0];
#pragma unroll
        for (int r = 1; r < 16; ++r) mx = fmaxf(mx, s[0][r]);
#pragma unroll
        for (int r = 0; r < 16; ++r) mx = fmaxf(mx, s[1][r]);
        mx = fmaxf(mx, __shfl_xor(mx, 32, 64));
        const float mn = fmaxf(m, mx);
        const float alpha = __builtin_amdgcn_exp2f(m - mn);
        m = mn;
        lsum *= alpha;
#pragma unroll
        for (int d = 0; d < DT; ++d) o[d] *= alpha;
        typedef float f32x2 __attribute__((ext_vector_type(2)));
        const f32x2 nm = {-m, -m};
        f32x2 ps2 = {0.f, 0.f};
#pragma unroll
        for (int ti = 0; ti < 2; ++ti)
#pragma unroll
            for (int r = 0; r < 16; r += 2) {
                f32x2 e = {s[ti][r], s[ti][r + 1]};
                e += nm;
                f32x2 p;
                p[0] = __builtin_amdgcn_exp2f(e[0]);
                p[1] = __builtin_amdgcn_exp2f(e[1]);
                s[ti][r] = p[0];
                s[ti][r + 1] = p[1];
                ps2 += p;
            }
        lsum += ps2[0] + ps2[1];
#pragma unroll
        for (int s2 = 0; s2 < 4; ++s2) {
            f16x8 pb;
#pragma unroll
            for (int j = 0; j < 8; ++j) pb[j] = (_Float16)s[s2 >> 1][(s2 & 1) * 8 + j];
#pragma unroll
            for (int d = 0; d < DT; ++d) {
                const char* vr = vb + s2 * 16 * VROW;
                const f16x8 va = __builtin_bit_cast(f16x8, __builtin_shufflevector(
                    __builtin_amdgcn_ds_read_tr16_b64_v4i16((tr_ptr)(vr + (vaddr[0] ^ (d << 6)))),
                    __builtin_amdgcn_ds_read_tr16_b64_v4i16((tr_ptr)(vr + (vaddr[1] ^ (d << 6)))), 0, 1, 2, 3, 4, 5, 6, 7));
                o[d] = __builtin_amdgcn_mfma_f32_32x32x16_f16(va, pb, o[d], 0, 0, 0);
            }
        }
        if (t + 1 < nt) LSTORE(buf ^ 1);
        __syncthreads();
    }
    if constexpr (NW == 8)
    for (int kx = 0; kx < k_origin; ++kx) {
        const __half* krow = base + E + (long)kx * ldq;
        float sdot = 0.f;
#pragma unroll
        for (int ks = 0; ks < KS; ++ks) {
            const f16x8 kv = *reinterpret_cast<const f16x8*>(krow + 16 * ks + 8 * hh);
#pragma unroll
            for (int j = 0; j < 8; ++j) sdot = fmaf((float)qf[ks][j], (float)kv[j], sdot);
        }
        sdot += __shfl_xor(sdot, 32, 64);
        const float mn = fmaxf(m, sdot);
        const float alpha = __builtin_amdgcn_exp2f(m - mn);
        const float pr = __builtin_amdgcn_exp2f(sdot - mn);
        m = mn;
        lsum = lsum * alpha + (hh == 0 ? pr : 0.f);
        const float p16 = (float)(_Float16)pr;
        const __half* vrow = base + 2 * E + (long)kx * ldq;
#pragma unroll
        for (int d = 0; d < DT; ++d)
#pragma unroll
            for (int g = 0; g < 4; ++g) {
                const f16x4 vv = *reinterpret_cast<const f16x4*>(vrow + d * 32 + 8 * g + 4 * hh);
#pragma unroll
                for (int k = 0; k < 4; ++k) o[d][g * 4 + k] = fmaf(p16, (float)vv[k], o[d][g * 4 + k] * alpha);
            }
    }
    const float ltot = lsum + __shfl_xor(lsum, 32, 64);
    const float inv = 1.0f / ltot;
#ifdef WC_NO_OSTAGE
    constexpr bool OSTAGE = false;
#else
    constexpr bool OSTAGE = NW == 8;
#endif
    if constexpr (OSTAGE) {
        constexpr int OPITCH = DH * 2 + 8;
        constexpr int CPR = DH / 8;
        char* stg = smem + wave * (32 * OPITCH);
    #pragma unroll
        for (int d = 0; d < DT; ++d)
    #pragma unroll
            for (int g = 0; g < 4; ++g) {
                __half hv[4];
    #pragma unroll
                for (int k = 0; k < 4; ++k) hv[k] = __float2half(o[d][g * 4 + k] * inv);
                *reinterpret_cast<uint2*>(stg + l31 * OPITCH + (d * 32 + 8 * g + 4 * hh) * 2) = *reinterpret_cast<uint2*>(hv);
            }
        asm volatile("s_waitcnt lgkmcnt(0)" ::: "memory");
        __builtin_amdgcn_wave_barrier();
        const int qw0 = q_origin + qb * (NW * 32) + wave * 32;
    #pragma unroll
        for (int i = 0; i < 32 * CPR / 64; ++i) {
            const int r = i * (64 / CPR) + lane / CPR, ch = lane % CPR;
            if (qw0 + r < L) {
                const uint2 lo2 = *reinterpret_cast<const uint2*>(stg + r * OPITCH + ch * 16);
                const uint2 hi2 = *reinterpret_cast<const uint2*>(stg + r * OPITCH + ch * 16 + 8);
                u32x4 v = {lo2.x, lo2.y, hi2.x, hi2.y};
                *reinterpret_cast<u32x4*>(out + ((long)b * L + qw0 + r) * E + (long)h * DH + ch * 8) = v;
            }
        }
    } else if (qrow < L) {
        __half* orow = out + ((long)b * L + qrow) * E + (long)h * DH;
#pragma unroll
        for (int d = 0; d < DT; ++d)
#pragma unroll
            for (int g = 0; g < 4; ++g) {
                __half hv[4];
#pragma unroll
                for (int k = 0; k < 4; ++k) hv[k] = __float2half(o[d][g * 4 + k] * inv);
                *reinterpret_cast<uint2*>(orow + d * 32 + 8 * g + 4 * hh) = *reinterpret_cast<uint2*>(hv);
            }
    }
    if (qrow < L) {
        if (out32) {
#pragma unroll
            for (int d = 0; d < DT; ++d)
#pragma unroll
                for (int g = 0; g < 4; ++g)
                    *reinterpret_cast<float4*>(out32 + ((long)b * L + qrow) * E + (long)h * DH + d * 32 + 8 * g + 4 * hh) =
                        make_float4(o[d][g * 4] * inv, o[d][g * 4 + 1] * inv, o[d][g * 4 + 2] * inv, o[d][g * 4 + 3] * inv);
        }
        if (hh == 0) lse[((long)b * H + h) * L + qrow] = m + log2f(ltot);
    }
}

template <int DH, int R>
__global__ __launch_bounds__(256, 2) void attn_mean_kernel(const __half* __restrict__ qkv,
                                                         const float* __restrict__ lse,
                                                         float* __restrict__ mean, int L, int H, int E, int origin,
                                                         int nt, int Bn) {
    constexpr int KS = DH / 16;
    constexpr int ROW = DH * 2 + 16;
    constexpr int TB = 128 * ROW;
    constexpr int CH = DH / 8;
    constexpr int NC = 128 * CH / 256;
    extern __shared__ __attribute__((aligned(16))) char smem[];
    constexpr int EDGE = 2 * TB + 512;
    constexpr int BUF = EDGE + (R > 0 ? 2 * R * DH * 2 + 32 : 0);

    const int tid = threadIdx.x, lane = tid & 63, wave = tid >> 6;
    const int hh = lane >> 5, l31 = lane & 31;
    const int wr = wave >> 1, wc = wave & 1;
    const int slot = blockIdx.x >> 3;
    const int b = (slot / (nt * nt)) * 8 + (blockIdx.x & 7);
    if (b >= Bn) return;
    const int rem = slot - (slot / (nt * nt)) * (nt * nt);
    const int k0 = origin + (rem % nt) * 128, q0 = origin + (rem / nt) * 128;
    const long ldq = 3L * E;
    const __half* base = qkv + (long)b * L * ldq;

    const bool edge_wg = R > 0 && (q0 == origin || k0 == origin);
    const bool edge_row = R > 0 && q0 == origin && tid < 128;
    const bool edge_col = R > 0 && k0 == origin && tid >= 128;
    const int e_which = tid / (origin * CH > 0 ? origin * CH : 1);
    const int e_rem = tid - e_which * origin * CH;
    const __half* e_src = base + (long)(e_rem / CH) * ldq + (e_which ? E : 0) + (e_rem % CH) * 8;
    const int e_dst = EDGE + (e_which * R * CH + e_rem) * 16;
    u32x4 rq[NC], rk[NC], re = {0u, 0u, 0u, 0u};
    float rl = 0.f;
#undef GLOAD
#define GLOAD(h_) \
    { \
        const int h__ = (h_); \
        _Pragma("unroll") \
        for (int i = 0; i < NC; ++i) { \
            const int c = tid + 256 * i; \
            int qr = q0 + c / CH, kr = k0 + c / CH; \
            if (qr > L - 1) qr = L - 1; \
            if (kr > L - 1) kr = L - 1; \
            rq[i] = *reinterpret_cast<const u32x4*>(base + (long)qr * ldq + h__ * DH + (c % CH) * 8); \
            rk[i] = *reinterpret_cast<const u32x4*>(base + (long)kr * ldq + E + h__ * DH + (c % CH) * 8); \
        } \
        if (tid < 128) { \
            int qr = q0 + tid; \
            if (qr > L - 1) qr = L - 1; \
            rl = lse[((long)b * H + h__) * L + qr]; \
        } \
        if constexpr (R > 0) \
            if (edge_wg) { \
                if (e_which < 2) re = *reinterpret_cast<const u32x4*>(e_src + h__ * DH); \
                if (tid >= 128 && tid < 128 + origin) rl = lse[((long)b * H + h__) * L + tid - 128]; \
            } \
    }
#undef LSTORE
#define LSTORE(buf_) \
    { \
        const int buf__ = (buf_); \
        char* qb = smem + buf__ * BUF; \
        _Pragma("unroll") \
        for (int i = 0; i < NC; ++i) { \
            const int c = tid + 256 * i; \
            *reinterpret_cast<u32x4*>(qb + (c / CH) * ROW + (c % CH) * 16) = rq[i]; \
            *reinterpret_cast<u32x4*>(qb + TB + (c / CH) * ROW + (c % CH) * 16) = rk[i]; \
        } \
        if (tid < 128) reinterpret_cast<float*>(qb + 2 * TB)[tid] = rl; \
        if constexpr (R > 0) \
            if (edge_wg) { \
                if (e_which < 2) *reinterpret_cast<u32x4*>(qb + e_dst) = re; \
                if (tid >= 128 && tid < 128 + origin) reinterpret_cast<float*>(qb + EDGE + 2 * R * DH * 2)[tid - 128] = rl; \
            } \
    }

    f32x16 acc[2][2];
#pragma unroll
    for (int i = 0; i < 2; ++i)
#pragma unroll
        for (int j = 0; j < 2; ++j)
#pragma unroll
            for (int r = 0; r < 16; ++r) acc[i][j][r] = 0.f;
    f16x8 b_aug;
#pragma unroll
    for (int j = 0; j < 8; ++j) b_aug[j] = (_Float16)((hh == 0 && j < 2) ? 1.0f : 0.0f);
    float eacc[R > 0 ? R : 1];
#pragma unroll
    for (int e = 0; e < (R > 0 ? R : 1); ++e) eacc[e] = 0.f;

    GLOAD(0);
    LSTORE(0);
    __syncthreads();
    for (int h = 0; h < H; ++h) {
        const int buf = h & 1;
        if (h + 1 < H) GLOAD(h + 1);
        const char* qb = smem + buf * BUF;
        const float* ls = reinterpret_cast<const float*>(qb + 2 * TB);
        f16x8 a_aug[2];
#pragma unroll
        for (int mi = 0; mi < 2; ++mi) {
            const float nl = -ls[wr * 64 + mi * 32 + l31];
            const _Float16 hi = (_Float16)nl;
            const _Float16 lo = (_Float16)(nl - (float)hi);
#pragma unroll
            for (int j = 0; j < 8; ++j) a_aug[mi][j] = (_Float16)0.0f;
            if (hh == 0) { a_aug[mi][0] = hi; a_aug[mi][1] = lo; }
        }
        f32x16 s[2][2];
        {
            f32x16 zero;
#pragma unroll
            for (int r = 0; r < 16; ++r) zero[r] = 0.f;
            s[0][0] = __builtin_amdgcn_mfma_f32_32x32x16_f16(a_aug[0], b_aug, zero, 0, 0, 0);
            s[0][1] = __builtin_amdgcn_mfma_f32_32x32x16_f16(a_aug[0], b_aug, zero, 0, 0, 0);
            s[1][0] = __builtin_amdgcn_mfma_f32_32x32x16_f16(a_aug[1], b_aug, zero, 0, 0, 0);
            s[1][1] = __builtin_amdgcn_mfma_f32_32x32x16_f16(a_aug[1], b_aug, zero, 0, 0, 0);
        }
        const char* As = qb + (wr * 64 + l31) * ROW + hh * 16;
        const char* Bs = qb + TB + (wc * 64 + l31) * ROW + hh * 16;
#pragma unroll
        for (int ks = 0; ks < KS; ++ks) {
            const f16x8 a0 = *reinterpret_cast<const f16x8*>(As + ks * 32);
            const f16x8 a1 = *reinterpret_cast<const f16x8*>(As + 32 * ROW + ks * 32);
            const f16x8 b0 = *reinterpret_cast<const f16x8*>(Bs + ks * 32);
            const f16x8 b1 = *reinterpret_cast<const f16x8*>(Bs + 32 * ROW + ks * 32);
            s[0][0] = __builtin_amdgcn_mfma_f32_32x32x16_f16(a0, b0, s[0][0], 0, 0, 0);
            s[0][1] = __builtin_amdgcn_mfma_f32_32x32x16_f16(a0, b1, s[0][1], 0, 0, 0);
            s[1][0] = __builtin_amdgcn_mfma_f32_32x32x16_f16(a1, b0, s[1][0], 0, 0, 0);
            s[1][1] = __builtin_amdgcn_mfma_f32_32x32x16_f16(a1, b1, s[1][1], 0, 0, 0);
        }
#pragma unroll
        for (int mi = 0; mi < 2; ++mi)
#pragma unroll
            for (int ni = 0; ni < 2; ++ni)
#pragma unroll
                for (int r = 0; r < 16; ++r) acc[mi][ni][r] += __builtin_amdgcn_exp2f(s[mi][ni][r]);
        if constexpr (R > 0)
        if (edge_row || edge_col) {
            const int t = tid & 127;
            const char* own = qb + (edge_row ? TB : 0) + t * ROW;
            const char* oth = qb + EDGE + (edge_row ? 0 : R * DH * 2);
            float sd[R];
#pragma unroll
            for (int e = 0; e < R; ++e) sd[e] = 0.f;
#pragma unroll
            for (int c = 0; c < CH; ++c) {
                const f16x8 ov = *reinterpret_cast<const f16x8*>(own + c * 16);
#pragma unroll
                for (int e = 0; e < R; ++e)
                    if (R == 1 || e < origin) {
                        const f16x8 xv = *reinterpret_cast<const f16x8*>(oth + e * DH * 2 + c * 16);
#pragma unroll
                        for (int j = 0; j < 4; ++j)
                            sd[e] = __builtin_amdgcn_fdot2(f16x2{xv[2 * j], xv[2 * j + 1]}, f16x2{ov[2 * j], ov[2 * j + 1]}, sd[e], false);
                    }
            }
            const float own_lse = ls[t];
            const float* els = reinterpret_cast<const float*>(qb + EDGE + 2 * R * DH * 2);
#pragma unroll
            for (int e = 0; e < R; ++e)
                if (R == 1 || e < origin) eacc[e] += __builtin_amdgcn_exp2f(sd[e] - (edge_row ? els[e] : own_lse));
        }
        if (h + 1 < H) LSTORE(buf ^ 1);
        __syncthreads();
    }
    const float invh = 1.0f / H;
    float* mb = mean + (long)b * L * L;
#pragma unroll
    for (int mi = 0; mi < 2; ++mi)
#pragma unroll
        for (int ni = 0; ni < 2; ++ni) {
            const int key = k0 + wc * 64 + ni * 32 + l31;
            if (key >= L) continue;
#pragma unroll
            for (int r = 0; r < 16; ++r) {
                const int q = q0 + wr * 64 + mi * 32 + (r & 3) + 8 * (r >> 2) + 4 * hh;
                if (q < L) mb[(long)q * L + key] = acc[mi][ni][r] * invh;
            }
        }
    if constexpr (R > 0)
    if (edge_row || edge_col) {
        const int t = tid & 127;
#pragma unroll
        for (int e = 0; e < R; ++e)
            if (R == 1 || e < origin) {
                if (edge_row) { if (k0 + t < L) mb[(long)e * L + k0 + t] = eacc[e] * invh; }
                else if (q0 + t < L) mb[(long)(q0 + t) * L + e] = eacc[e] * invh;
            }
    }
    if (R > 0 && q0 == origin && k0 == origin && tid < origin * origin) {
        const int qe = tid / origin, ke = tid - qe * origin;
        float a = 0.f;
        for (int h = 0; h < H; ++h) {
            const __half* qr = base + (long)qe * ldq + h * DH;
            const __half* kr = base + (long)ke * ldq + E + h * DH;
            float sd = 0.f;
#pragma unroll
            for (int c = 0; c < CH; ++c) {
                const f16x8 xv = *reinterpret_cast<const f16x8*>(qr + c * 8);
                const f16x8 kv = *reinterpret_cast<const f16x8*>(kr + c * 8);
#pragma unroll
                for (int j = 0; j < 8; ++j) sd = fmaf((float)xv[j], (float)kv[j], sd);
            }
            a += __builtin_amdgcn_exp2f(sd - lse[((long)b * H + h) * L + qe]);
        }
        mb[(long)qe * L + ke] = a * invh;
    }
}

static int attn_origin(int L) {
    const int r = L % 128;
    return (L >= 128 && r > 0 && r <= ATT_EDGE_MAX) ? r : 0;
}

extern "C" int wc_attn_fwd(const void* qkv, void* out, float* out32, float* lse, int B, int L, int H, int DH,
                           void* stream) {
    const int E = H * DH;
    WC_CHECK_ARG(qkv && out && lse && B > 0 && L > 0 && H > 0, "wc_attn_fwd: bad argument");
    WC_CHECK_ARG(DH == 64 || DH == 32, "wc_attn_fwd: head dim must be 32 or 64 (got %d)", DH);
    WC_CHECK_ARG(((uintptr_t)qkv | (uintptr_t)out | (uintptr_t)out32) % 16 == 0, "wc_attn_fwd: operands must be 16-byte aligned");
    WC_CHECK_ARG(E % 8 == 0 && B <= 65535 && H <= 65535 && (long)wc_cdiv(L, 128) * H * (B + 7) < (1L << 30),
                 "wc_attn_fwd: bad shape");
    const size_t lds = DH == 64 ? 2 * (64 * (64 * 2 + 16) + 64 * 128) : 2 * (64 * (32 * 2 + 16) + 64 * 64);
    const int NWv = (DH == 64 && (long)wc_cdiv(L, 256) * H * B >= 512) ? 8 : 4;
    const int nthr = NWv * 64;
    int r = attn_origin(L);
    if (r && ((size_t)L + 4 + 16 + (nthr / (DH / 8)) * DH) * 4 > lds) r = 0;
    const int kr = (NWv == 8 && L >= 64 && L % 64 > 0 && L % 64 <= ATT_EDGE_MAX) ? L % 64 : 0;
    const int nqb = wc_cdiv(L - r, NWv * 32);
    dim3 grid((unsigned)(nqb * H * ((B + 7) / 8 * 8) + r * H * B));
    hipStream_t st = (hipStream_t)stream;
    const int pr = wc_prof_begin(stream);
    if (DH == 64 && NWv == 8)
        hipLaunchKernelGGL((attn_fwd_kernel<64, 8>), grid, dim3(512), lds, st, (const __half*)qkv, (__half*)out, out32, lse, L, H,
                           E, r, nqb, B, kr);
    else if (DH == 64)
        hipLaunchKernelGGL((attn_fwd_kernel<64, 4>), grid, dim3(256), lds, st, (const __half*)qkv, (__half*)out, out32, lse, L, H,
                           E, r, nqb, B, kr);
    else
        hipLaunchKernelGGL((attn_fwd_kernel<32, 4>), grid, dim3(256), lds, st, (const __half*)qkv, (__half*)out, out32, lse, L, H,
                           E, r, nqb, B, kr);
    wc_prof_end(pr, DH == 64 ? (NWv == 8 ? "attn_fwd_kernel<64, 8>" : "attn_fwd_kernel<64, 4>") : "attn_fwd_kernel<32, 4>",
                4.0 * B * H * (double)L * L * DH, stream);
    WC_LAUNCH_CHECK("attn_fwd_kernel");
    return WC_OK;
}

extern "C" int wc_attn_mean(const void* qkv, const float* lse, float* mean, int B, int L, int H, int DH,
                            void* stream) {
    const int E = H * DH;
    WC_CHECK_ARG(qkv && lse && mean && B > 0 && L > 0 && H > 0, "wc_attn_mean: bad argument");
    WC_CHECK_ARG(DH == 64 || DH == 32, "wc_attn_mean: head dim must be 32 or 64 (got %d)", DH);
    WC_CHECK_ARG((uintptr_t)qkv % 16 == 0, "wc_attn_mean: qkv must be 16-byte aligned");
    const int r = attn_origin(L);
    const int nt = wc_cdiv(L - r, 128);
    dim3 grid((unsigned)(nt * nt * ((B + 7) / 8 * 8)));
    hipStream_t st = (hipStream_t)stream;
    const int rcap = r == 0 ? 0 : (r == 1 ? 1 : ATT_EDGE_MAX);
    const size_t lds = 2 * ((size_t)2 * 128 * (DH * 2 + 16) + 512 + (rcap ? 2 * rcap * DH * 2 + 32 : 0));
    static bool lds_attr_set = false;
    if (!lds_attr_set) {
#define WC_MEAN_ATTR(DH_, R_) \
    (hipFuncSetAttribute((const void*)attn_mean_kernel<DH_, R_>, hipFuncAttributeMaxDynamicSharedMemorySize, 80 * 1024) == hipSuccess)
        WC_CHECK_ARG(WC_MEAN_ATTR(64, 0) && WC_MEAN_ATTR(64, 1) && WC_MEAN_ATTR(64, ATT_EDGE_MAX) && WC_MEAN_ATTR(32, 0) &&
                     WC_MEAN_ATTR(32, 1) && WC_MEAN_ATTR(32, ATT_EDGE_MAX), "wc_attn_mean: cannot reserve 80 KiB of LDS");
#undef WC_MEAN_ATTR
        lds_attr_set = true;
    }
    const int pr = wc_prof_begin(stream);
#define WC_MEAN_LAUNCH(DH_, R_) \
    hipLaunchKernelGGL((attn_mean_kernel<DH_, R_>), grid, dim3(256), lds, st, (const __half*)qkv, lse, mean, L, H, E, r, nt, B)
    if (DH == 64) {
        if (r == 0) WC_MEAN_LAUNCH(64, 0); else if (r == 1) WC_MEAN_LAUNCH(64, 1); else WC_MEAN_LAUNCH(64, ATT_EDGE_MAX);
    } else {
        if (r == 0) WC_MEAN_LAUNCH(32, 0); else if (r == 1) WC_MEAN_LAUNCH(32, 1); else WC_MEAN_LAUNCH(32, ATT_EDGE_MAX);
    }
#undef WC_MEAN_LAUNCH
    static const char* const mean_names[2][3] = {{"attn_mean_kernel<64, 0>", "attn_mean_kernel<64, 1>", "attn_mean_kernel<64, 8>"},
                                                 {"attn_mean_kernel<32, 0>", "attn_mean_kernel<32, 1>", "attn_mean_kernel<32, 8>"}};
    wc_prof_end(pr, mean_names[DH == 64 ? 0 : 1][r == 0 ? 0 : (r == 1 ? 1 : 2)], 2.0 * B * H * (double)L * L * DH, stream);
    WC_LAUNCH_CHECK("attn_mean_kernel");
    return WC_OK;
}
```

### weclip-vit-comer_amd/gradcam_engine.py

```python
import torch

from . import _lib as L
from . import ops
from .ops import F16, F32, Split
from .clip import vit_engine as VE

def _logit_scale(clip_model):
    p = clip_model.logit_scale
    key = (p.data_ptr(), p._version)
    cached = getattr(clip_model, "_logit_scale_host", None)
    if cached is None or cached[0] != key:
        cached = (key, float(p.detach().exp().item()))
        clip_model._logit_scale_host = cached
    return cached[1]


GRAD_SCALE = 4096.0


class _BwdPack:

    def __init__(self, blk):
        t = lambda w: ops.split_f16(w.detach().float().t().contiguous())
        self.pjT = t(blk.mlp.c_proj.weight)
        self.fcT = t(blk.mlp.c_fc.weight)
        self.outT = t(blk.attn.out_proj.weight)
        self.w_in = blk.attn.in_proj_weight.detach().float().contiguous()
        self.ln2_w = blk.ln_2.weight.detach().float().contiguous()


class LastLayerState:

    def __init__(self, clip_model, x2, mean, keep, B, Lq):
        self.m, self.x2, self.mean, self.keep, self.B, self.L = clip_model, x2, mean, keep, B, Lq
        blk = clip_model.visual.transformer.resblocks[-1]
        if getattr(blk, "_bwd_pack", None) is None or blk._bwd_pack.w_in.device != x2.device:
            blk._bwd_pack = _BwdPack(blk)
        self.bw = blk._bwd_pack
        self.blk = blk

    def _head(self, text_hat, text_idx, n_text, pair_img, pair_cls, Tmax):
        v = self.m.visual
        B, Lq = self.B, self.L
        E, Ed = v.proj.shape
        P = pair_img.numel()
        dev = self.x2.device
        nchunk = (Lq + 15) // 16
        partial = torch.empty(B * nchunk * E, device=dev, dtype=F32)
        probs = torch.zeros(P, Tmax, device=dev, dtype=F32)
        df = torch.empty(P, E, device=dev, dtype=F32)
        L.lib().wc_cam_head(L.ptr(self.x2, F32), L.ptr(v.ln_post.weight.detach().float(), F32),
                            L.ptr(v.ln_post.bias.detach().float(), F32),
                            L.ptr(v.proj.detach().float().contiguous(), F32), L.ptr(text_hat, F32),
                            L.ptr(text_idx, torch.int32), L.ptr(n_text, torch.int32),
                            L.ptr(pair_img, torch.int32), L.ptr(pair_cls, torch.int32),
                            _logit_scale(self.m), L.ptr(partial), L.ptr(probs),
                            L.ptr(df), B, P, Lq, E, Ed, Tmax, L.stream())
        return probs, df

    def class_probs(self, text):
        dev = self.x2.device
        T = text.shape[0]
        that = (text / text.norm(dim=1, keepdim=True)).contiguous()
        idx = torch.arange(T, dtype=torch.int32, device=dev).repeat(self.B, 1).contiguous()
        nt = torch.full((self.B,), T, dtype=torch.int32, device=dev)
        img = torch.arange(self.B, dtype=torch.int32, device=dev)
        cls = torch.zeros(self.B, dtype=torch.int32, device=dev)
        probs, _ = self._head(that, idx, nt, img, cls, T)
        return probs

    def grad_cam(self, text_hat, text_idx, n_text, pair_img, pair_cls, Tmax):
        lib = L.lib()
        k, bw = self.keep, self.bw
        B, Lq = self.B, self.L
        E = self.x2.shape[1]
        H = self.blk.attn.num_heads
        DH = E // H
        P = pair_img.numel()
        M = P * Lq
        dev = self.x2.device
        st = L.stream
        probs, df = self._head(text_hat, text_idx, n_text, pair_img, pair_cls, Tmax)
        v = self.m.visual
        dx2 = torch.empty(M, E, device=dev, dtype=F32)
        from . import config
        ex = config.exact()
        dx2s = Split(torch.empty(M, E, device=dev, dtype=F16), torch.empty(M, E, device=dev, dtype=F16) if ex else None)
        lib.wc_lnpost_bwd(L.ptr(df), L.ptr(self.x2), L.ptr(v.ln_post.weight.detach().float(), F32),
                          GRAD_SCALE, L.ptr(pair_img), L.ptr(dx2), L.ptr(dx2s.hi), L.ptr(dx2s.lo), P, Lq, E,
                          st())
        du = Split(torch.empty(M, 4 * E, device=dev, dtype=F16), torch.empty(M, 4 * E, device=dev, dtype=F16) if ex else None)
        ops.gemm(dx2s, bw.pjT, M, 4 * E, E, out16=du.hi, out16lo=du.lo, act=4, aux=k["u32"],
                 rowmap=pair_img, rpg=Lq, ldaux=4 * E)
        da2 = torch.empty(M, E, device=dev, dtype=F32)
        ops.gemm(du, bw.fcT, M, E, 4 * E, out32=da2)
        g16 = torch.empty(M, E, device=dev, dtype=F16)
        lib.wc_ln2_bwd_add(L.ptr(da2), L.ptr(dx2), L.ptr(k["x1"]), L.ptr(bw.ln2_w), GRAD_SCALE,
                           L.ptr(pair_img), L.ptr(g16), P, Lq, E, st())
        do16 = torch.empty(M, E, device=dev, dtype=F16)
        ops.gemm(g16, bw.outT, M, E, E, out16=do16)
        ws = torch.empty(4, P, H, Lq, device=dev, dtype=F32)
        c = torch.empty(P, 3 * E, device=dev, dtype=F32)
        lib.wc_attn_bwd_colsum(L.ptr(k["qkv"]), L.ptr(do16), L.ptr(k["o32"]), L.ptr(k["lse"]),
                               L.ptr(pair_img), L.ptr(ws[0]), L.ptr(ws[1]), L.ptr(ws[2]), L.ptr(ws[3]),
                               L.ptr(c), P, Lq, H, DH, st())
        w = torch.empty(P, E, device=dev, dtype=F32)
        ws2 = torch.empty(16 * P * E, device=dev, dtype=F32)
        lib.wc_rowvec_matmul(L.ptr(c), L.ptr(bw.w_in), L.ptr(w), L.ptr(ws2), P, 3 * E, E, 1.0 / (Lq - 1), st())
        cams = torch.empty(P, Lq - 1, device=dev, dtype=F32)
        lib.wc_cam_map(L.ptr(k["a32"]), L.ptr(w), L.ptr(pair_img), L.ptr(cams), P, Lq, E, st())
        return cams, probs, w


def last_layer_forward(clip_model, rows, B, Lq, want_mean=True):
    blk = clip_model.visual.transformer.resblocks[-1]
    keep = {}
    x2, mean = VE.run_block(blk.pack(), rows, B, Lq, want_mean=want_mean, keep=keep, tag=b"@vit_attn")
    return LastLayerState(clip_model, x2, mean, keep, B, Lq)
```

### weclip-vit-comer_amd/ops.py

```python
import ctypes
import math

import torch

from . import _lib as L

F16 = torch.float16
F32 = torch.float32
LOG2E = 1.4426950408889634


class KernelTimer:

    active = False

    @staticmethod
    def enable(stride=1):
        L.lib().cdll.wc_prof_enable(int(stride))
        KernelTimer.active = bool(stride)
        if not stride:
            L.lib().cdll.wc_prof_tag(None)

    @staticmethod
    def tag(name):
        if KernelTimer.active:
            L.lib().cdll.wc_prof_tag(name)

    @staticmethod
    def summary():
        import ctypes
        buf = ctypes.create_string_buffer(1 << 16)
        L.lib().cdll.wc_prof_report(buf, len(buf))
        out = {}
        for line in buf.value.decode().splitlines():
            name, n, ms, work, est, nbytes = line.split("\t")
            out[name] = {"ms": float(ms), "launches": int(n), "work": float(work), "est_ms": float(est), "bytes": float(nbytes)}
        return out


class Split:
    __slots__ = ("hi", "lo")

    def __init__(self, hi, lo=None):
        self.hi, self.lo = hi, lo


def split_f16(x, with_lo=False):
    L.require_gpu()
    x = x.detach().float().contiguous()
    hi = torch.empty(x.shape, device=x.device, dtype=F16)
    lo = torch.empty(x.shape, device=x.device, dtype=F16) if with_lo else None
    L.lib().wc_split_f16(L.ptr(x, F32, "x"), L.ptr(hi), L.ptr(lo), x.numel(), L.stream())
    return Split(hi, lo)


def gemm(a, w, M, N, K, *, lda=None, ldw=None, bias=None, resid=None, ldr=None, sR=None,
         out32=None, out16=None, out16lo=None, ldc=None, act=0, round16=False, scale=1.0,
         scale_cols=0, batch=1, sA=0, sW=0, sC=0, pre32=None, aux=None, rowmap=None, rpg=0,
         ldaux=0, auxh=None, cscale=None, sCS=0, zdiv=None, sA2=0, sW2=0, sC2=0, sB2=0, sX2=0):
    a = a if isinstance(a, Split) else Split(a)
    w = w if isinstance(w, Split) else Split(w)
    segs = [(a.hi, w.hi)]
    if a.lo is not None:
        segs.append((a.lo, w.hi))
    if w.lo is not None:
        segs.append((a.hi, w.lo))
    lda = K if lda is None else lda
    ldw = K if ldw is None else ldw
    ldc = N if ldc is None else ldc
    ap = [L.ptr(s[0], F16, "A") for s in segs] + [None] * (3 - len(segs))
    wp = [L.ptr(s[1], F16, "W") for s in segs] + [None] * (3 - len(segs))
    ldr = ldc if ldr is None else ldr
    sR = sC if sR is None else sR
    L.lib().wc_gemm_f16_grouped(ap[0], ap[1], ap[2], wp[0], wp[1], wp[2], len(segs), M, N, K, lda, ldw,
                                batch, sA, sW, sC, L.ptr(bias, F32, "bias"), L.ptr(resid, F32, "resid"),
                                ldr, sR, L.ptr(out32, F32, "out32"), L.ptr(out16, F16, "out16"),
                                L.ptr(out16lo, F16, "out16lo"), ldc, act, 1 if round16 else 0,
                                float(scale), scale_cols, L.ptr(pre32, F32, "pre32"), L.ptr(aux, F32, "aux"),
                                L.ptr(rowmap, torch.int32, "rowmap"), rpg, ldaux, L.ptr(auxh, F16, "auxh"),
                                L.ptr(cscale, F32, "cscale"), sCS, batch if zdiv is None else zdiv, sA2, sW2, sC2, sB2,
                                sX2, L.stream())


def gemm_row_ok(M, N, K):
    return N <= 256 and N % 4 == 0 and K in (128, 256) and M > 0


def gemm_row(a16, w16, M, N, K, *, lda=None, ldw=None, bias=None, cscale=None, act=0, aux=None, auxh=None, ldaux=0, resid=None,
             ldr=None, out32=None, out16=None, pre32=None, ldc=None, ldc16=None, ln=(), eps=1e-5):
    lda = K if lda is None else lda
    ldw = K if ldw is None else ldw
    ldc = N if ldc is None else ldc
    ldr = ldc if ldr is None else ldr
    ldc16 = ldc if ldc16 is None else ldc16
    lnp = [None] * 6
    for i, (gam, bet, out) in enumerate(ln):
        lnp[3 * i:3 * i + 3] = [L.ptr(gam, F32, "ln.weight"), L.ptr(bet, F32, "ln.bias"), L.ptr(out, F16, "ln.out")]
    L.lib().wc_gemm_row_f16(L.ptr(a16, F16, "A"), lda, L.ptr(w16, F16, "W"), ldw, M, N, K, L.ptr(bias, F32, "bias"),
                            L.ptr(cscale, F32, "cscale"), act, L.ptr(aux, F32, "aux"), L.ptr(auxh, F16, "auxh"), ldaux,
                            L.ptr(resid, F32, "resid"), ldr, L.ptr(out32, F32, "out32"), L.ptr(out16, F16, "out16"),
                            L.ptr(pre32, F32, "pre32"), ldc, ldc16, lnp[0], lnp[1], lnp[2], lnp[3], lnp[4], lnp[5], float(eps), L.stream())


def gemm_row_grouped(a16, w16, M, N, K, groups, *, lda=None, ldw=None, bias=None, act=0, auxh=None, ldaux=0, out32=None, out16=None,
                     ldc=None, ldc16=None, gA=0, gW=0, gB=0, gC=0, gX=0):
    lda = K if lda is None else lda
    ldw = K if ldw is None else ldw
    ldc = N if ldc is None else ldc
    ldc16 = ldc if ldc16 is None else ldc16
    L.lib().wc_gemm_row_f16_grouped(L.ptr(a16, F16, "A"), lda, L.ptr(w16, F16, "W"), ldw, M, N, K, L.ptr(bias, F32, "bias"), act,
                                    L.ptr(auxh, F16, "auxh"), ldaux, L.ptr(out32, F32, "out32"), L.ptr(out16, F16, "out16"), ldc, ldc16,
                                    groups, gA, gW, gB, gC, gX, L.stream())


def layernorm(x, weight, bias, *, eps=1e-5, want32=False, want16=True, with_lo=False, rows=None,
              D=None, ldx=None):
    D = x.shape[-1] if D is None else D
    rows = x.numel() // D if rows is None else rows
    ldx = D if ldx is None else ldx
    dev = x.device
    y32 = torch.empty(rows, D, device=dev, dtype=F32) if want32 else None
    hi = torch.empty(rows, D, device=dev, dtype=F16) if want16 else None
    lo = torch.empty(rows, D, device=dev, dtype=F16) if (want16 and with_lo) else None
    L.lib().wc_layernorm(L.ptr(x, F32, "x"), ldx, L.ptr(weight, F32, "ln.weight"),
                         L.ptr(bias, F32, "ln.bias"), eps, L.ptr(y32), L.ptr(hi), L.ptr(lo), rows, D,
                         L.stream())
    return y32, (Split(hi, lo) if want16 else None)


def attention(qkv16, B, Lq, H, DH, want_mean=True, want_o32=False):
    E = H * DH
    dev = qkv16.device
    lib = L.lib()
    o16 = torch.empty(B * Lq, E, device=dev, dtype=F16)
    lse = torch.empty(B, H, Lq, device=dev, dtype=F32)
    o32 = torch.empty(B * Lq, E, device=dev, dtype=F32) if want_o32 else None
    lib.wc_attn_fwd(L.ptr(qkv16, F16, "qkv"), L.ptr(o16), L.ptr(o32), L.ptr(lse), B, Lq, H, DH, L.stream())
    mean = None
    if want_mean:
        mean = torch.empty(B, Lq, Lq, device=dev, dtype=F32)
        lib.wc_attn_mean(L.ptr(qkv16), L.ptr(lse), L.ptr(mean), B, Lq, H, DH, L.stream())
    if want_o32:
        return o16, lse, mean, o32
    return o16, lse, mean


def attention_causal(qkv16, B, Lq, H, DH, want_mean=True, want_o32=False):
    E = H * DH
    dev = qkv16.device
    o16 = torch.empty(B * Lq, E, device=dev, dtype=F16)
    lse = torch.empty(B, H, Lq, device=dev, dtype=F32)
    o32 = torch.empty(B * Lq, E, device=dev, dtype=F32) if want_o32 else None
    mean = torch.empty(B, Lq, Lq, device=dev, dtype=F32) if want_mean else None
    L.lib().wc_attn_fwd_causal(L.ptr(qkv16, F16, "qkv"), L.ptr(o16), L.ptr(o32), L.ptr(lse), L.ptr(mean), B, Lq, H, DH,
                               L.stream())
    if want_o32:
        return o16, lse, mean, o32
    return o16, lse, mean


def text_embed(tokens, tok_emb, pos, L_used):
    N, Lctx = tokens.shape
    V, W = tok_emb.shape
    dev = tokens.device
    x = torch.empty(N * L_used, W, device=dev, dtype=F32) if L_used else None
    flags = torch.empty(N + 1, device=dev, dtype=torch.int32)
    L.lib().wc_text_embed(L.ptr(tokens, torch.int32, "tokens"), N, Lctx, L.ptr(tok_emb, F32, "token_embedding"), V,
                          L.ptr(pos, F32, "positional_embedding"), W, L_used, L.ptr(x), L.ptr(flags[:N]), L.ptr(flags[N:]),
                          L.stream())
    return x, flags[:N], flags[N:]


def text_pool(x, eot, N, Lq, ln_w, ln_b, proj, eps=1e-5):
    W, Ed = proj.shape
    feat = torch.empty(N, Ed, device=x.device, dtype=F32)
    L.lib().wc_text_pool(L.ptr(x, F32, "x"), L.ptr(eot, torch.int32, "eot"), N, Lq, W, L.ptr(ln_w, F32, "ln_final.weight"),
                         L.ptr(ln_b, F32, "ln_final.bias"), float(eps), L.ptr(proj, F32, "text_projection"), Ed, L.ptr(feat),
                         L.stream())
    return feat


def text_zeroshot(feat, C, T):
    Ed = feat.shape[-1]
    out = torch.empty(C, Ed, device=feat.device, dtype=F32)
    L.lib().wc_text_zeroshot(L.ptr(feat, F32, "features"), C, T, Ed, L.ptr(out), L.stream())
    return out


def q_scale(DH):
    return LOG2E / math.sqrt(DH)



def attention_bwd(qkv16, do16, o32, lse, B, Lq, H, DH, with_lo=True):
    E = H * DH
    dev = qkv16.device
    Lp = (Lq + 63) // 64 * 64
    ws = torch.empty(3, B * H * DH * Lp, device=dev, dtype=F16)
    delta = torch.empty(B * H * Lq, device=dev, dtype=F32)
    d = Split(torch.empty(B * Lq, 3 * E, device=dev, dtype=F16),
              torch.empty(B * Lq, 3 * E, device=dev, dtype=F16) if with_lo else None)
    L.lib().wc_attn_bwd(L.ptr(qkv16, F16, "qkv"), L.ptr(do16, F16, "dO"), L.ptr(o32, F32, "o32"), L.ptr(lse, F32, "lse"),
                        L.ptr(ws[0]), L.ptr(ws[1]), L.ptr(ws[2]), L.ptr(delta), L.ptr(d.hi), L.ptr(d.lo), B, Lq, Lp,
                        H, DH, L.stream())
    return d


def transpose_f16(src, R, C, *, ld=None, batch=1, sSrc=0, with_lo=False, scale=1.0, oR=None, ones_row=False):
    ld = C if ld is None else ld
    oR = R if oR is None else oR
    K = (batch - 1) * oR + R
    Kp = (batch * oR + 63) // 64 * 64
    dev = src.device
    alloc = torch.zeros if Kp != K else torch.empty
    rows = C + 1 if ones_row else C
    hi = alloc(rows, Kp, device=dev, dtype=F16)
    lo = alloc(rows, Kp, device=dev, dtype=F16) if with_lo else None
    if ones_row:
        if oR != R:
            raise RuntimeError("ones_row needs densely packed batches")
        hi[C, :K] = 1.0
        if lo is not None:
            lo[C].zero_()
    f32 = src.dtype == F32
    L.lib().wc_transpose_f16(L.ptr(src, F32 if f32 else F16, "src"), 1 if f32 else 0, ld, sSrc, L.ptr(hi), L.ptr(lo),
                             Kp, oR, batch, R, C, float(scale), L.stream())
    return Split(hi, lo), Kp


_ZEROS = {}


def wgrad_tiles(N, K, bias=True):
    kt = K // 128 if (bias and K % 128 == 0) else (K + (1 if bias else 0) + 127) // 128
    return ((N + 127) // 128) * kt


def wgrad_partials(dy16, x16, M, N, K, *, lda=None, ldx=None, slices=1, bias=True, xmap=None, groups=1, gA=0, gX=0, queue=None):
    L.require_gpu()
    lda = N if lda is None else lda
    ldx = K if ldx is None else ldx
    dev = dy16.device
    mslice = (-(-M // slices) + 63) // 64 * 64
    ns = -(-M // mslice)
    K1 = K + (1 if bias else 0)
    part = torch.empty((ns, N, K1) if groups == 1 else (groups, ns, N, K1), device=dev, dtype=F32)
    rpg, gs, off = xmap if xmap is not None else (max(M, 64), 0, 0)
    if queue is not None:
        queue.append(((dy16, x16, part), [L.ptr(dy16, F16, "dY").value, L.ptr(x16, F16, "X").value, part.data_ptr(), M, N, K, lda,
                                          ldx, rpg, gs, off, mslice, 1 if bias else 0, groups, gA, gX]))
        return part, ns
    L.lib().wc_gemm_km_f16_grouped(L.ptr(dy16, F16, "dY"), lda, L.ptr(x16, F16, "X"), ldx, L.ptr(_zeros(dev)), M, N, K, rpg, gs, off,
                                   mslice, 1 if bias else 0, L.ptr(part), groups, gA, gX, L.stream())
    return part, ns


def _zeros(dev):
    z = _ZEROS.get(dev)
    if z is None:
        z = _ZEROS[dev] = torch.zeros(64, device=dev, dtype=F16)
    return z


def wgrad_launch(queue):
    jobs = list(queue)
    del queue[:]
    if jobs:
        flat = [v for _, fields in jobs for v in fields]
        L.lib().wc_gemm_km_f16_multi((ctypes.c_int64 * len(flat))(*flat), len(jobs), L.ptr(_zeros(jobs[0][0][0].device)), L.stream())


def colsum(src, R, C, *, ld=None, alpha=1.0, round16=False, out=None):
    ld = C if ld is None else ld
    dev = src.device
    part = torch.empty(((R + 255) // 256) * C, device=dev, dtype=F32)
    out = torch.empty(C, device=dev, dtype=F32) if out is None else out
    f32 = src.dtype == F32
    L.lib().wc_colsum(L.ptr(src, F32 if f32 else F16, "src"), 1 if f32 else 0, ld, L.ptr(part), L.ptr(out, F32), R, C,
                      float(alpha), 1 if round16 else 0, L.stream())
    return out


def layernorm_bwd(dy, x, w, *, add=None, want32=True, want16=False, out_scale=1.0, alpha=1.0, eps=1e-5, dgb=None):
    rows, D = x.shape
    dev = x.device
    dx32 = torch.empty(rows, D, device=dev, dtype=F32) if want32 else None
    dx16 = torch.empty(rows, D, device=dev, dtype=F16) if want16 else None
    part = torch.empty(((rows + 15) // 16) * 2 * D, device=dev, dtype=F32)
    if dgb is None:
        dgb = torch.empty(2, D, device=dev, dtype=F32)
    fn = L.lib().wc_layernorm_bwd_h if dy.dtype == F16 else L.lib().wc_layernorm_bwd
    fn(L.ptr(dy, dy.dtype, "dy"), L.ptr(x, F32, "x"), L.ptr(w, F32, "w"), L.ptr(add, F32, "add"), eps,
       L.ptr(dx32), L.ptr(dx16), float(out_scale), L.ptr(part), L.ptr(dgb), float(alpha), rows, D, L.stream())
    return dx32, dx16, dgb


def layernorm_bwd2(dya, wa, dyb, wb, x, *, add=None, want32=True, want16=False, out_scale=1.0, alpha=1.0, eps=1e-5, dgba=None, dgbb=None):
    rows, D = x.shape
    dev = x.device
    dx32 = torch.empty(rows, D, device=dev, dtype=F32) if want32 else None
    dx16 = torch.empty(rows, D, device=dev, dtype=F16) if want16 else None
    part = torch.empty(min((rows + 15) // 16, 2048) * 4 * D, device=dev, dtype=F32)
    dgba = torch.empty(2, D, device=dev, dtype=F32) if dgba is None else dgba
    dgbb = torch.empty(2, D, device=dev, dtype=F32) if dgbb is None else dgbb
    L.lib().wc_layernorm_bwd2_h(L.ptr(dya, F16, "dya"), L.ptr(wa, F32, "wa"), L.ptr(dyb, F16, "dyb"), L.ptr(wb, F32, "wb"),
                                L.ptr(x, F32, "x"), L.ptr(add, F32, "add"), eps, L.ptr(dx32), L.ptr(dx16), float(out_scale),
                                L.ptr(part), L.ptr(dgba), L.ptr(dgbb), float(alpha), rows, D, L.stream())
    return dx32, dx16, dgba, dgbb


def sigmoid_gram_bwd(dAP, AP, scale=1.0, with_lo=True):
    B, n, _ = AP.shape
    np_ = (n + 63) // 64 * 64
    alloc = torch.zeros if np_ != n else torch.empty
    s = Split(alloc(B, n, np_, device=AP.device, dtype=F16),
              alloc(B, n, np_, device=AP.device, dtype=F16) if with_lo else None)
    L.lib().wc_sigmoid_gram_bwd(L.ptr(dAP, F32, "dAP"), L.ptr(AP, F32, "AP"), L.ptr(s.hi), L.ptr(s.lo), B, n, np_,
                                float(scale), L.stream())
    return s


def colscale_split(x, cs, rows_per_batch, want32=True, with_lo=True, alpha=1.0):
    rows, C = x.shape
    dev = x.device
    out32 = torch.empty(rows, C, device=dev, dtype=F32) if want32 else None
    s = Split(torch.empty(rows, C, device=dev, dtype=F16), torch.empty(rows, C, device=dev, dtype=F16) if with_lo else None)
    L.lib().wc_colscale_split(L.ptr(x, F32, "x"), L.ptr(cs, F32, "cs"), L.ptr(out32), L.ptr(s.hi), L.ptr(s.lo), rows, C,
                              rows_per_batch, float(alpha), L.stream())
    return out32, s


class WeightCache:

    def __init__(self):
        self.key = None
        self.versions = None
        self.views = {}

    def refresh(self, named, exact, force=False, lo_names=()):
        L.require_gpu()
        lo_names = frozenset(lo_names)
        named = [(n, list(t) if isinstance(t, (list, tuple)) else [t]) for n, t in named]
        flat = [t for _, ts in named for t in ts]
        key = tuple((n, tuple((t.data_ptr(), tuple(t.shape)) for t in ts)) for n, ts in named) + (bool(exact), lo_names)
        if key != self.key:
            dev = flat[0].device
            tot = sum(t.numel() for t in flat)
            totT = sum(ts[0].shape[1] * ((sum(t.shape[0] for t in ts) + 63) // 64 * 64) for _, ts in named)
            self.hi = torch.empty(tot, device=dev, dtype=F16)
            self.lo = torch.empty(tot, device=dev, dtype=F16) if (exact or lo_names) else None
            self.hiT = torch.zeros(totT, device=dev, dtype=F16)
            self.loT = torch.zeros(totT, device=dev, dtype=F16) if exact else None
            rows, self.views, o, oT = [], {}, 0, 0
            for n, ts in named:
                R, C = sum(t.shape[0] for t in ts), ts[0].shape[1]
                ldT = (R + 63) // 64 * 64
                has_lo = exact or n in lo_names
                hi, hiT = self.hi[o:o + R * C].view(R, C), self.hiT[oT:oT + C * ldT].view(C, ldT)
                lo = self.lo[o:o + R * C].view(R, C) if has_lo else None
                loT = self.loT[oT:oT + C * ldT].view(C, ldT) if exact else None
                r0 = 0
                for t in ts:
                    if t.shape[1] != C or (len(ts) > 1 and r0 % 4):
                        raise RuntimeError("WeightCache: stacked matrices need equal widths and row counts that are multiples of 4")
                    rows.append([t.data_ptr(), hi.data_ptr() + 2 * r0 * C, (lo.data_ptr() + 2 * r0 * C) if has_lo else 0,
                                 hiT.data_ptr() + 2 * r0, (loT.data_ptr() + 2 * r0) if exact else 0, t.shape[0], C, ldT])
                    r0 += t.shape[0]
                self.views[n] = (Split(hi, lo), Split(hiT, loT), ldT)
                o += R * C
                oT += C * ldT
            self.table = torch.tensor(rows, dtype=torch.int64).pin_memory().to(dev, non_blocking=True)
            self.count = len(rows)
            self.key, self.versions = key, None
        versions = tuple(t._version for t in flat)
        if force or versions != self.versions:
            L.lib().wc_convert_weights(L.ptr(self.table, torch.int64, "table"), self.count, 32, L.stream())
            self.versions = versions

    def w(self, name):
        return self.views[name][0]

    def wT(self, name):
        return self.views[name][1], self.views[name][2]
```

Baseline: 1351 images/sec.

## Accumulate weighted attention-mean maps in-kernel instead of storing per-layer maps

Adds an accumulating variant of the attention-mean kernel that writes the weighted, CLS-stripped patch-to-patch map directly into a single running affinity buffer for the last 8 layers. The separate per-layer Lq×Lq map tensors and the later affinity-weight kernel that reads and averages them are no longer needed. The column sums (c1) are recomputed from the accumulated W by a new small reduction kernel. This cuts memory traffic and allocations in the no-grad CAM path. The cost is a read-modify-write of W per layer and a peeled last-head loop in the kernel.

```diff
diff --git a/include/weclip_hip.h b/include/weclip_hip.h
--- a/include/weclip_hip.h
+++ b/include/weclip_hip.h
@@ -106,6 +106,9 @@
                 void* stream);
 int wc_attn_mean(const void* qkv, const float* lse, float* mean, int B, int L, int H, int DH,
                  void* stream);
+int wc_attn_mean_acc_supported(int L);
+int wc_attn_mean_acc(const void* qkv, const float* lse, float* W, float weight, int first, int B, int L, int H,
+                     int DH, void* stream);
 
 int wc_patchify(const float* img, void* hi, void* lo, int B, int H, int W, int P, void* stream);
 int wc_cls_rows(float* x, const float* cls, const float* pos0, int B, int L, int E, void* stream);
@@ -135,6 +138,7 @@
 int wc_aff_fused_supported(int hw);
 int wc_aff_weight_c1(const float* const* h_maps, int nmaps, const float* wgt, const float* seg, float* W, float* c1,
                      float* ws, int B, int L, void* stream);
+int wc_aff_c1_from_w(const float* W, float* c1, float* ws, int B, int hw, void* stream);
 int wc_aff_sinkhorn_step(const float* W, const float* c, float* r, float* c_next, float* ws, int B, int hw, int last,
                          void* stream);
 int wc_aff_tsym_apply(const float* W, const float* r, const float* c, const float* X, float* out, float* y1, float* ws,
diff --git a/weclip-vit-comer_amd/WeCLIP_model/model_attn_aff_voc.py b/weclip-vit-comer_amd/WeCLIP_model/model_attn_aff_voc.py
--- a/weclip-vit-comer_amd/WeCLIP_model/model_attn_aff_voc.py
+++ b/weclip-vit-comer_amd/WeCLIP_model/model_attn_aff_voc.py
@@ -5,6 +5,7 @@
 import torch.nn as nn
 
 from .. import cam_pipeline as CP
+from .. import ops
 from ..clip import clip_tool as CT
 from ..clip import vit_engine as VE
 from ..clip.clip import load as clip_load
@@ -48,6 +49,7 @@
     seg_trans_last = 6
     seg_trans_after = 15000
     val_runs_cam = True
+    accumulate_maps = True
     fg_names, bg_names = "new_class_names", "BACKGROUND_CATEGORY"
 
     def __init__(self, num_classes=None, clip_model=None, embedding_dim=256, in_channels=512,
@@ -103,9 +105,15 @@
         first = 12 - n
         return [i >= first for i in range(11)]
 
-    def encode(self, img, seg_trans, x16=None, want_maps=True):
+    def encode(self, img, seg_trans, x16=None, want_maps=True, acc=None):
         need = self._maps_needed(seg_trans) if want_maps else [False] * 11
-        return VE.encode_blocks(self.encoder.visual, img, need, x16)
+        return VE.encode_blocks(self.encoder.visual, img, need, x16, acc=acc)
+
+    def _map_accumulator(self, img, seg_trans, want_cam):
+        Lq = (img.shape[2] // 16) * (img.shape[3] // 16) + 1
+        if not self.accumulate_maps or seg_trans or not want_cam or not img.is_cuda or not ops.MapAccumulator.supported(Lq):
+            return None
+        return ops.MapAccumulator(img.shape[0], Lq, 8, img.device)
 
     def forward(self, img, img_names="2007_000032", mode="train", labels=None, plan=None, sizes=None):
         B, _, H, W = img.shape
@@ -120,7 +128,8 @@
         x16 = VE.X16Stack(self.encoder.visual.transformer.layers - 1) if (hip_head or comer_tokens) else None
         with torch.no_grad():
             want_cam = not (mode == "val" and not self.val_runs_cam)
-            xs, maps, _, Lq = self.encode(img, seg_trans, x16, want_maps=want_cam)
+            acc = self._map_accumulator(img, seg_trans, want_cam)
+            xs, maps, _, Lq = self.encode(img, seg_trans, x16, want_maps=want_cam, acc=acc)
         if hip_head:
             drop = self.head_engine.draw_dropout(B, img.device) if self.training else None
             fork = self.fork_head and want_cam and img.is_cuda
@@ -139,7 +148,7 @@
 
                 with torch.no_grad():
                     cam_labels = self.cam_labels(img, xs[-1], maps, joined_attn_pred if seg_trans else None, img_names, labels, mode,
-                                                 seg_trans, h, w, plan=plan, sizes=sizes)
+                                                 seg_trans, h, w, plan=plan, sizes=sizes, acc=acc)
                 main.wait_stream(side)
                 return seg, cam_labels, attn_pred
             seg, attn_pred = HeadFunction.apply(self.head_engine, x16, B, Lq, h, w, drop, *self.head_engine.params())
@@ -153,7 +162,8 @@
                 with torch.cuda.stream(side):
                     seg, attn_pred = self._module_head(img, xs, x16, comer_tokens, B, Lq, h, w)
                 with torch.no_grad():
-                    cam_labels = self.cam_labels(img, xs[-1], maps, None, img_names, labels, mode, seg_trans, h, w, plan=plan, sizes=sizes)
+                    cam_labels = self.cam_labels(img, xs[-1], maps, None, img_names, labels, mode, seg_trans, h, w, plan=plan, sizes=sizes,
+                                                 acc=acc)
                 main.wait_stream(side)
                 return seg, cam_labels, attn_pred
             seg, attn_pred = self._module_head(img, xs, x16, comer_tokens, B, Lq, h, w)
@@ -161,7 +171,7 @@
             return seg, None, attn_pred
         with torch.no_grad():
             cam_labels = self.cam_labels(img, xs[-1], maps, attn_pred.detach(), img_names, labels, mode,
-                                         seg_trans, h, w, plan=plan, sizes=sizes)
+                                         seg_trans, h, w, plan=plan, sizes=sizes, acc=acc)
         return seg, cam_labels, attn_pred
 
     def side_streams(self):
@@ -189,7 +199,8 @@
             attn_pred = torch.sigmoid(f.transpose(2, 1).bmm(f))
         return seg, attn_pred
 
-    def cam_labels(self, img, last_rows, maps, attn_pred, img_names, labels, mode, seg_trans, h, w, plan=None, sizes=None):
+    def cam_labels(self, img, last_rows, maps, attn_pred, img_names, labels, mode, seg_trans, h, w, plan=None, sizes=None,
+                   acc=None):
         if self.bg_text_features is None or self.fg_text_features is None:
             raise RuntimeError("WeCLIP needs text_features=(bg, fg) (see __init__): pass them, or call "
                                "install_dropin(reference_root=<reference checkout>) before constructing WeCLIP so that "
@@ -209,7 +220,7 @@
         text_hat = CT.normalised_text(self.fg_text_features, self.bg_text_features, dev)
         R, _, _, _ = CT.batch_refined_cams(self.encoder, last_rows, maps, attn_pred if seg_trans else None,
                                            plan, text_hat, h, w, self.cam_threshold, seg_trans,
-                                           self.seg_trans_last)
+                                           self.seg_trans_last, acc=acc)
         C = plan.K + 1
         if mode == "train" or all(tuple(s) == (H, W) for s in sizes):
             cams = CP.upsample_with_bg(R, plan.nk, h, w, H, W, C)
diff --git a/weclip-vit-comer_amd/cam_pipeline.py b/weclip-vit-comer_amd/cam_pipeline.py
--- a/weclip-vit-comer_amd/cam_pipeline.py
+++ b/weclip-vit-comer_amd/cam_pipeline.py
@@ -35,7 +35,20 @@
     return (hw + 31) // 32
 
 
-def affinity_weight(maps, seg=None, seg_trans=False, n_last=6, keep=None, return_c1=False):
+def affinity_weight(maps, seg=None, seg_trans=False, n_last=6, keep=None, return_c1=False, acc=None):
+    if acc is not None:
+        if seg_trans or acc.n_layers != 8:
+            raise RuntimeError("affinity_weight: an accumulator serves the normal branch (the last 8 maps) only")
+        W = acc.result()
+        B, hw, _ = W.shape
+        if not return_c1:
+            return W
+        if not fused_ok(hw):
+            return W, None
+        c1 = torch.empty(B, hw, device=W.device, dtype=F32)
+        ws = torch.empty(B * ((hw + 7) // 8) * hw, device=W.device, dtype=F32)
+        L.lib().wc_aff_c1_from_w(L.ptr(W), L.ptr(c1), L.ptr(ws), B, hw, L.stream())
+        return W, c1
     sel = maps[-n_last:] if seg_trans else maps[-8:]
     B, Lq, _ = sel[0].shape
     hw = Lq - 1
diff --git a/weclip-vit-comer_amd/clip/clip_tool.py b/weclip-vit-comer_amd/clip/clip_tool.py
--- a/weclip-vit-comer_amd/clip/clip_tool.py
+++ b/weclip-vit-comer_amd/clip/clip_tool.py
@@ -124,12 +124,14 @@
 
 
 def batch_refined_cams(clip_model, last_rows, maps11, seg_attn, plan, text_hat, h, w, thr,
-                       seg_trans, n_last, keep=None):
+                       seg_trans, n_last, keep=None, acc=None):
     B, Lq = plan.B, h * w + 1
-    st = last_layer_forward(clip_model, last_rows, B, Lq)
+    if acc is not None and seg_trans:
+        raise RuntimeError("batch_refined_cams: the seg-trans branch needs the maps themselves, not their accumulated mean")
+    st = last_layer_forward(clip_model, last_rows, B, Lq, acc=acc)
     maps = list(maps11) + [st.mean]
     need = maps[-n_last:] if seg_trans else maps[-8:]
-    if any(m is None for m in need):
+    if acc is None and any(m is None for m in need):
         raise RuntimeError("attention maps needed by the affinity were not computed")
     if callable(seg_attn):
         if seg_trans:
@@ -139,7 +141,7 @@
             return R, cams, probs, st
         seg_attn = None
     cams, probs, _ = st.grad_cam(text_hat, plan.text_idx, plan.n_text, plan.pair_img, plan.pair_cls, plan.Tmax)
-    W, c1 = CP.affinity_weight(maps, seg_attn, seg_trans, n_last, keep=keep, return_c1=True)
+    W, c1 = CP.affinity_weight(maps, seg_attn, seg_trans, n_last, keep=keep, return_c1=True, acc=acc)
     R = CP.refine(W, cams, plan.pair_img, plan.pair_slot, plan.K, h, w, thr, c1=c1)
     return R, cams, probs, st
 
diff --git a/weclip-vit-comer_amd/clip/vit_engine.py b/weclip-vit-comer_amd/clip/vit_engine.py
--- a/weclip-vit-comer_amd/clip/vit_engine.py
+++ b/weclip-vit-comer_amd/clip/vit_engine.py
@@ -43,7 +43,7 @@
         return Split(self.big[i], self.big_lo[i] if self.big_lo is not None else None)
 
 
-def run_block(pk, x, B, L, want_mean=True, keep=None, x16_out=None, tag=None, causal=False):
+def run_block(pk, x, B, L, want_mean=True, keep=None, x16_out=None, tag=None, causal=False, acc=None):
     M, E, H, DH = B * L, pk.E, pk.H, pk.DH
     dev = x.device
     ex = pk.exact
@@ -54,10 +54,13 @@
     ops.gemm(a, pk.in_w, M, 3 * E, E, bias=pk.in_b, out16=qkv, scale=ops.q_scale(DH), scale_cols=E)
     o32 = None
     attn = ops.attention_causal if causal else ops.attention
+    if acc is not None and causal:
+        raise RuntimeError("run_block: the causal attention has no accumulating form")
+    kw = {} if acc is None else {"acc": acc}
     if keep is not None:
-        o16, lse, mean, o32 = attn(qkv, B, L, H, DH, want_mean=want_mean, want_o32=True)
+        o16, lse, mean, o32 = attn(qkv, B, L, H, DH, want_mean=want_mean, want_o32=True, **kw)
     else:
-        o16, lse, mean = attn(qkv, B, L, H, DH, want_mean=want_mean)
+        o16, lse, mean = attn(qkv, B, L, H, DH, want_mean=want_mean, **kw)
     x1 = torch.empty(M, E, device=dev, dtype=F32)
     ops.gemm(o16, pk.out_w, M, E, E, bias=pk.out_b, resid=x, out32=x1, round16=True)
     if tag:
@@ -81,11 +84,12 @@
     return x2, mean
 
 
-def encode_blocks(vis, img, need, x16=None):
+def encode_blocks(vis, img, need, x16=None, acc=None):
     rows, B, Lq = vis.embed(img)
     xs, maps = [], []
     for i in range(vis.transformer.layers - 1):
-        rows, m = run_block(vis.transformer.resblocks[i].pack(), rows, B, Lq, want_mean=need[i], x16_out=x16, tag=b"@vit_attn")
+        rows, m = run_block(vis.transformer.resblocks[i].pack(), rows, B, Lq, want_mean=need[i], x16_out=x16, tag=b"@vit_attn",
+                            acc=acc)
         xs.append(rows)
         maps.append(m)
     return xs, maps, B, Lq
diff --git a/weclip-vit-comer_amd/csrc/affinity.hip b/weclip-vit-comer_amd/csrc/affinity.hip
--- a/weclip-vit-comer_amd/csrc/affinity.hip
+++ b/weclip-vit-comer_amd/csrc/affinity.hip
@@ -210,6 +210,25 @@
             cs += v;
         }
         colpart[((long)b * nblk + blk) * hw + j] = cs;
+    }
+}
+
+__global__ __launch_bounds__(256) void aff_colpart_w_kernel(const float* __restrict__ W, float* __restrict__ colpart, int hw) {
+    const int blk = blockIdx.x, b = blockIdx.y, nblk = gridDim.x;
+    const int i0 = blk * AF_RPBW, i1 = min(i0 + AF_RPBW, hw);
+    for (int j = threadIdx.x * 4; j < hw; j += 1024) {
+        float4 v[AF_RPBW];
+#pragma unroll
+        for (int r = 0; r < AF_RPBW; ++r)
+            v[r] = *reinterpret_cast<const float4*>(W + ((long)b * hw + min(i0 + r, i1 - 1)) * hw + j);
+        float4 cs = make_float4(0.f, 0.f, 0.f, 0.f);
+#pragma unroll
+        for (int r = 0; r < AF_RPBW; ++r) {
+            const bool in = i0 + r < i1;
+            cs.x = in ? cs.x + v[r].x : cs.x; cs.y = in ? cs.y + v[r].y : cs.y;
+            cs.z = in ? cs.z + v[r].z : cs.z; cs.w = in ? cs.w + v[r].w : cs.w;
+        }
+        *reinterpret_cast<float4*>(colpart + ((long)b * nblk + blk) * hw + j) = cs;
     }
 }
 
@@ -564,6 +583,20 @@
     return WC_OK;
 }
 
+extern "C" int wc_aff_c1_from_w(const float* W, float* c1, float* ws, int B, int hw, void* stream) {
+    WC_CHECK_ARG(W && c1 && ws && B > 0 && B <= 65535 && aff_fused_ok(hw), "wc_aff_c1_from_w: bad argument");
+    WC_CHECK_ARG(((uintptr_t)W | (uintptr_t)ws) % 16 == 0, "wc_aff_c1_from_w: W and ws must be 16-byte aligned");
+    const int nblk = wc_cdiv(hw, AF_RPBW);
+    hipStream_t st = (hipStream_t)stream;
+    const int pr = wc_prof_begin(stream);
+    hipLaunchKernelGGL(aff_colpart_w_kernel, dim3(nblk, B), dim3(256), 0, st, W, ws, hw);
+    wc_prof_end(pr, "aff_colpart_w_kernel", (double)B * hw * hw * 4.0, stream);
+    WC_LAUNCH_CHECK("aff_colpart_w_kernel");
+    hipLaunchKernelGGL(aff_colreduce_kernel, dim3(wc_cdiv(hw, 256), B), dim3(256), 0, st, ws, nullptr, nullptr, c1, hw, 1, nblk, 0);
+    WC_LAUNCH_CHECK("aff_colreduce_kernel");
+    return WC_OK;
+}
+
 extern "C" int wc_aff_sinkhorn_step(const float* W, const float* c, float* r, float* c_next, float* ws, int B, int hw,
                                     int last, void* stream) {
     WC_CHECK_ARG(W && c && r && ws && (last || c_next) && B > 0 && B <= 65535 && aff_fused_ok(hw), "wc_aff_sinkhorn_step: bad argument");
diff --git a/weclip-vit-comer_amd/csrc/attention.hip b/weclip-vit-comer_amd/csrc/attention.hip
--- a/weclip-vit-comer_amd/csrc/attention.hip
+++ b/weclip-vit-comer_amd/csrc/attention.hip
@@ -1,5 +1,6 @@
 #include "common.h"
 #include <stdlib.h>
+#include <type_traits>
 
 typedef _Float16 f16x8 __attribute__((ext_vector_type(8)));
 typedef _Float16 f16x4 __attribute__((ext_vector_type(4)));
@@ -342,11 +343,12 @@
     }
 }
 
-template <int DH, int R>
+template <int DH, int R, bool ACC>
 __global__ __launch_bounds__(256, 2) void attn_mean_kernel(const __half* __restrict__ qkv,
                                                          const float* __restrict__ lse,
                                                          float* __restrict__ mean, int L, int H, int E, int origin,
-                                                         int nt, int Bn) {
+                                                         int nt, int Bn, float wgt, int first) {
+    constexpr int E0 = ACC ? 1 : 0;
     constexpr int KS = DH / 16;
     constexpr int ROW = DH * 2 + 16;
     constexpr int TB = 128 * ROW;
@@ -432,13 +434,32 @@
     float eacc[R > 0 ? R : 1];
 #pragma unroll
     for (int e = 0; e < (R > 0 ? R : 1); ++e) eacc[e] = 0.f;
+    const int hw = L - 1;
+    float* wb = mean + (long)b * hw * hw;
+    f32x16 wold[ACC ? 2 : 1][2];
+#undef WLOAD
+#define WLOAD(mi_) \
+    { \
+        _Pragma("unroll") \
+        for (int ni = 0; ni < 2; ++ni) { \
+            const int key = min(k0 + wc * 64 + ni * 32 + l31, L - 1); \
+            _Pragma("unroll") \
+            for (int r = 0; r < 16; ++r) { \
+                const int q = min(q0 + wr * 64 + (mi_) * 32 + (r & 3) + 8 * (r >> 2) + 4 * hh, L - 1); \
+                wold[mi_][ni][r] = wb[(long)(q - 1) * hw + key - 1]; \
+            } \
+        } \
+    }
 
     GLOAD(0);
     LSTORE(0);
     __syncthreads();
-    for (int h = 0; h < H; ++h) {
+    auto head_step = [&](const int h, auto peeled) {
+        constexpr bool LAST = decltype(peeled)::value;
         const int buf = h & 1;
-        if (h + 1 < H) GLOAD(h + 1);
+        if (!LAST && h + 1 < H) GLOAD(h + 1);
+        if constexpr (LAST)
+            if (!first) { WLOAD(0); WLOAD(1); }
         const char* qb = smem + buf * BUF;
         const float* ls = reinterpret_cast<const float*>(qb + 2 * TB);
         f16x8 a_aug[2];
@@ -451,35 +472,42 @@
             for (int j = 0; j < 8; ++j) a_aug[mi][j] = (_Float16)0.0f;
             if (hh == 0) { a_aug[mi][0] = hi; a_aug[mi][1] = lo; }
         }
-        f32x16 s[2][2];
-        {
-            f32x16 zero;
-#pragma unroll
-            for (int r = 0; r < 16; ++r) zero[r] = 0.f;
-            s[0][0] = __builtin_amdgcn_mfma_f32_32x32x16_f16(a_aug[0], b_aug, zero, 0, 0, 0);
-            s[0][1] = __builtin_amdgcn_mfma_f32_32x32x16_f16(a_aug[0], b_aug, zero, 0, 0, 0);
-            s[1][0] = __builtin_amdgcn_mfma_f32_32x32x16_f16(a_aug[1], b_aug, zero, 0, 0, 0);
-            s[1][1] = __builtin_amdgcn_mfma_f32_32x32x16_f16(a_aug[1], b_aug, zero, 0, 0, 0);
-        }
         const char* As = qb + (wr * 64 + l31) * ROW + hh * 16;
         const char* Bs = qb + TB + (wc * 64 + l31) * ROW + hh * 16;
-#pragma unroll
-        for (int ks = 0; ks < KS; ++ks) {
-            const f16x8 a0 = *reinterpret_cast<const f16x8*>(As + ks * 32);
-            const f16x8 a1 = *reinterpret_cast<const f16x8*>(As + 32 * ROW + ks * 32);
-            const f16x8 b0 = *reinterpret_cast<const f16x8*>(Bs + ks * 32);
-            const f16x8 b1 = *reinterpret_cast<const f16x8*>(Bs + 32 * ROW + ks * 32);
-            s[0][0] = __builtin_amdgcn_mfma_f32_32x32x16_f16(a0, b0, s[0][0], 0, 0, 0);
-            s[0][1] = __builtin_amdgcn_mfma_f32_32x32x16_f16(a0, b1, s[0][1], 0, 0, 0);
-            s[1][0] = __builtin_amdgcn_mfma_f32_32x32x16_f16(a1, b0, s[1][0], 0, 0, 0);
-            s[1][1] = __builtin_amdgcn_mfma_f32_32x32x16_f16(a1, b1, s[1][1], 0, 0, 0);
-        }
-#pragma unroll
-        for (int mi = 0; mi < 2; ++mi)
-#pragma unroll
-            for (int ni = 0; ni < 2; ++ni)
-#pragma unroll
-                for (int r = 0; r < 16; ++r) acc[mi][ni][r] += __builtin_amdgcn_exp2f(s[mi][ni][r]);
+        constexpr int MG = LAST ? 1 : 2;
+#pragma unroll
+        for (int m0 = 0; m0 < 2; m0 += MG) {
+            f32x16 s[MG][2];
+            {
+                f32x16 zero;
+#pragma unroll
+                for (int r = 0; r < 16; ++r) zero[r] = 0.f;
+#pragma unroll
+                for (int i = 0; i < MG; ++i) {
+                    s[i][0] = __builtin_amdgcn_mfma_f32_32x32x16_f16(a_aug[m0 + i], b_aug, zero, 0, 0, 0);
+                    s[i][1] = __builtin_amdgcn_mfma_f32_32x32x16_f16(a_aug[m0 + i], b_aug, zero, 0, 0, 0);
+                }
+            }
+#pragma unroll
+            for (int ks = 0; ks < KS; ++ks) {
+                f16x8 a[MG];
+#pragma unroll
+                for (int i = 0; i < MG; ++i) a[i] = *reinterpret_cast<const f16x8*>(As + (m0 + i) * 32 * ROW + ks * 32);
+                const f16x8 b0 = *reinterpret_cast<const f16x8*>(Bs + ks * 32);
+                const f16x8 b1 = *reinterpret_cast<const f16x8*>(Bs + 32 * ROW + ks * 32);
+#pragma unroll
+                for (int i = 0; i < MG; ++i) {
+                    s[i][0] = __builtin_amdgcn_mfma_f32_32x32x16_f16(a[i], b0, s[i][0], 0, 0, 0);
+                    s[i][1] = __builtin_amdgcn_mfma_f32_32x32x16_f16(a[i], b1, s[i][1], 0, 0, 0);
+                }
+            }
+#pragma unroll
+            for (int i = 0; i < MG; ++i)
+#pragma unroll
+                for (int ni = 0; ni < 2; ++ni)
+#pragma unroll
+                    for (int r = 0; r < 16; ++r) acc[m0 + i][ni][r] += __builtin_amdgcn_exp2f(s[i][ni][r]);
+        }
         if constexpr (R > 0)
         if (edge_row || edge_col) {
             const int t = tid & 127;
@@ -493,7 +521,7 @@
                 const f16x8 ov = *reinterpret_cast<const f16x8*>(own + c * 16);
 #pragma unroll
                 for (int e = 0; e < R; ++e)
-                    if (R == 1 || e < origin) {
+                    if (e >= E0 && (R == 1 || e < origin)) {
                         const f16x8 xv = *reinterpret_cast<const f16x8*>(oth + e * DH * 2 + c * 16);
 #pragma unroll
                         for (int j = 0; j < 4; ++j)
@@ -504,13 +532,27 @@
             const float* els = reinterpret_cast<const float*>(qb + EDGE + 2 * R * DH * 2);
 #pragma unroll
             for (int e = 0; e < R; ++e)
-                if (R == 1 || e < origin) eacc[e] += __builtin_amdgcn_exp2f(sd[e] - (edge_row ? els[e] : own_lse));
-        }
-        if (h + 1 < H) LSTORE(buf ^ 1);
-        __syncthreads();
+                if (e >= E0 && (R == 1 || e < origin)) eacc[e] += __builtin_amdgcn_exp2f(sd[e] - (edge_row ? els[e] : own_lse));
+        }
+        if (!LAST && h + 1 < H) LSTORE(buf ^ 1);
+        if (!LAST) __syncthreads();
+    };
+    if constexpr (ACC) {
+        for (int h = 0; h + 1 < H; ++h) head_step(h, std::false_type{});
+        head_step(H - 1, std::true_type{});
+    } else {
+        for (int h = 0; h < H; ++h) head_step(h, std::false_type{});
     }
     const float invh = 1.0f / H;
     float* mb = mean + (long)b * L * L;
+    auto put = [&](int q, int key, float v) {
+        if constexpr (ACC) {
+            float* w = wb + (long)(q - 1) * hw + key - 1;
+            *w = fmaf(wgt, v, first ? 0.f : *w);
+        } else {
+            mb[(long)q * L + key] = v;
+        }
+    };
 #pragma unroll
     for (int mi = 0; mi < 2; ++mi)
 #pragma unroll
@@ -520,20 +562,24 @@
 #pragma unroll
             for (int r = 0; r < 16; ++r) {
                 const int q = q0 + wr * 64 + mi * 32 + (r & 3) + 8 * (r >> 2) + 4 * hh;
-                if (q < L) mb[(long)q * L + key] = acc[mi][ni][r] * invh;
+                if (q >= L) continue;
+                if constexpr (ACC)
+                    wb[(long)(q - 1) * hw + key - 1] = fmaf(wgt, acc[mi][ni][r] * invh, first ? 0.f : wold[mi][ni][r]);
+                else
+                    mb[(long)q * L + key] = acc[mi][ni][r] * invh;
             }
         }
     if constexpr (R > 0)
     if (edge_row || edge_col) {
         const int t = tid & 127;
 #pragma unroll
-        for (int e = 0; e < R; ++e)
+        for (int e = E0; e < R; ++e)
             if (R == 1 || e < origin) {
-                if (edge_row) { if (k0 + t < L) mb[(long)e * L + k0 + t] = eacc[e] * invh; }
-                else if (q0 + t < L) mb[(long)(q0 + t) * L + e] = eacc[e] * invh;
-            }
-    }
-    if (R > 0 && q0 == origin && k0 == origin && tid < origin * origin) {
+                if (edge_row) { if (k0 + t < L) put(e, k0 + t, eacc[e] * invh); }
+                else if (q0 + t < L) put(q0 + t, e, eacc[e] * invh);
+            }
+    }
+    if (R > 0 && q0 == origin && k0 == origin && tid < origin * origin && tid / origin >= E0 && tid % origin >= E0) {
         const int qe = tid / origin, ke = tid - qe * origin;
         float a = 0.f;
         for (int h = 0; h < H; ++h) {
@@ -549,7 +595,7 @@
             }
             a += __builtin_amdgcn_exp2f(sd - lse[((long)b * H + h) * L + qe]);
         }
-        mb[(long)qe * L + ke] = a * invh;
+        put(qe, ke, a * invh);
     }
 }
 
@@ -606,7 +652,7 @@
     static bool lds_attr_set = false;
     if (!lds_attr_set) {
 #define WC_MEAN_ATTR(DH_, R_) \
-    (hipFuncSetAttribute((const void*)attn_mean_kernel<DH_, R_>, hipFuncAttributeMaxDynamicSharedMemorySize, 80 * 1024) == hipSuccess)
+    (hipFuncSetAttribute((const void*)attn_mean_kernel<DH_, R_, false>, hipFuncAttributeMaxDynamicSharedMemorySize, 80 * 1024) == hipSuccess)
         WC_CHECK_ARG(WC_MEAN_ATTR(64, 0) && WC_MEAN_ATTR(64, 1) && WC_MEAN_ATTR(64, ATT_EDGE_MAX) && WC_MEAN_ATTR(32, 0) &&
                      WC_MEAN_ATTR(32, 1) && WC_MEAN_ATTR(32, ATT_EDGE_MAX), "wc_attn_mean: cannot reserve 80 KiB of LDS");
 #undef WC_MEAN_ATTR
@@ -614,7 +660,8 @@
     }
     const int pr = wc_prof_begin(stream);
 #define WC_MEAN_LAUNCH(DH_, R_) \
-    hipLaunchKernelGGL((attn_mean_kernel<DH_, R_>), grid, dim3(256), lds, st, (const __half*)qkv, lse, mean, L, H, E, r, nt, B)
+    hipLaunchKernelGGL((attn_mean_kernel<DH_, R_, false>), grid, dim3(256), lds, st, (const __half*)qkv, lse, mean, L, H, E, r, nt, B, \
+                       0.f, 1)
     if (DH == 64) {
         if (r == 0) WC_MEAN_LAUNCH(64, 0); else if (r == 1) WC_MEAN_LAUNCH(64, 1); else WC_MEAN_LAUNCH(64, ATT_EDGE_MAX);
     } else {
@@ -627,3 +674,43 @@
     WC_LAUNCH_CHECK("attn_mean_kernel");
     return WC_OK;
 }
+
+extern "C" int wc_attn_mean_acc_supported(int L) { return L >= 2 ? 1 : 0; }
+
+extern "C" int wc_attn_mean_acc(const void* qkv, const float* lse, float* W, float weight, int first, int B, int L, int H,
+                                int DH, void* stream) {
+    const int E = H * DH;
+    WC_CHECK_ARG(qkv && lse && W && B > 0 && L >= 2 && H > 0, "wc_attn_mean_acc: bad argument");
+    WC_CHECK_ARG(DH == 64 || DH == 32, "wc_attn_mean_acc: head dim must be 32 or 64 (got %d)", DH);
+    WC_CHECK_ARG((uintptr_t)qkv % 16 == 0, "wc_attn_mean_acc: qkv must be 16-byte aligned");
+    const int r = attn_origin(L) > 1 ? attn_origin(L) : 1;
+    const int nt = wc_cdiv(L - r, 128);
+    dim3 grid((unsigned)(nt * nt * ((B + 7) / 8 * 8)));
+    hipStream_t st = (hipStream_t)stream;
+    const int rcap = r == 1 ? 0 : ATT_EDGE_MAX;
+    const size_t lds = 2 * ((size_t)2 * 128 * (DH * 2 + 16) + 512 + (rcap ? 2 * rcap * DH * 2 + 32 : 0));
+    static bool lds_attr_set = false;
+    if (!lds_attr_set) {
+#define WC_MEAN_ATTR(DH_, R_) \
+    (hipFuncSetAttribute((const void*)attn_mean_kernel<DH_, R_, true>, hipFuncAttributeMaxDynamicSharedMemorySize, 80 * 1024) == hipSuccess)
+        WC_CHECK_ARG(WC_MEAN_ATTR(64, 0) && WC_MEAN_ATTR(64, ATT_EDGE_MAX) && WC_MEAN_ATTR(32, 0) && WC_MEAN_ATTR(32, ATT_EDGE_MAX),
+                     "wc_attn_mean_acc: cannot reserve 80 KiB of LDS");
+#undef WC_MEAN_ATTR
+        lds_attr_set = true;
+    }
+    const int pr = wc_prof_begin(stream);
+#define WC_MEAN_LAUNCH(DH_, R_) \
+    hipLaunchKernelGGL((attn_mean_kernel<DH_, R_, true>), grid, dim3(256), lds, st, (const __half*)qkv, lse, W, L, H, E, r, nt, B, \
+                       weight, first ? 1 : 0)
+    if (DH == 64) {
+        if (r == 1) WC_MEAN_LAUNCH(64, 0); else WC_MEAN_LAUNCH(64, ATT_EDGE_MAX);
+    } else {
+        if (r == 1) WC_MEAN_LAUNCH(32, 0); else WC_MEAN_LAUNCH(32, ATT_EDGE_MAX);
+    }
+#undef WC_MEAN_LAUNCH
+    static const char* const acc_names[2][2] = {{"attn_mean_acc_kernel<64, 0>", "attn_mean_acc_kernel<64, 8>"},
+                                                {"attn_mean_acc_kernel<32, 0>", "attn_mean_acc_kernel<32, 8>"}};
+    wc_prof_end(pr, acc_names[DH == 64 ? 0 : 1][r == 1 ? 0 : 1], 2.0 * B * H * (double)(L - 1) * (L - 1) * DH, stream);
+    WC_LAUNCH_CHECK("attn_mean_acc_kernel");
+    return WC_OK;
+}
diff --git a/weclip-vit-comer_amd/gradcam_engine.py b/weclip-vit-comer_amd/gradcam_engine.py
--- a/weclip-vit-comer_amd/gradcam_engine.py
+++ b/weclip-vit-comer_amd/gradcam_engine.py
@@ -112,8 +112,8 @@
         return cams, probs, w
 
 
-def last_layer_forward(clip_model, rows, B, Lq, want_mean=True):
+def last_layer_forward(clip_model, rows, B, Lq, want_mean=True, acc=None):
     blk = clip_model.visual.transformer.resblocks[-1]
     keep = {}
-    x2, mean = VE.run_block(blk.pack(), rows, B, Lq, want_mean=want_mean, keep=keep, tag=b"@vit_attn")
+    x2, mean = VE.run_block(blk.pack(), rows, B, Lq, want_mean=want_mean, keep=keep, tag=b"@vit_attn", acc=acc)
     return LastLayerState(clip_model, x2, mean, keep, B, Lq)
diff --git a/weclip-vit-comer_amd/ops.py b/weclip-vit-comer_amd/ops.py
--- a/weclip-vit-comer_amd/ops.py
+++ b/weclip-vit-comer_amd/ops.py
@@ -128,7 +128,31 @@
     return y32, (Split(hi, lo) if want16 else None)
 
 
-def attention(qkv16, B, Lq, H, DH, want_mean=True, want_o32=False):
+class MapAccumulator:
+
+    def __init__(self, B, Lq, n_layers, device):
+        self.B, self.Lq, self.n_layers, self.done = B, Lq, n_layers, 0
+        self.weight = 1.0 / n_layers
+        self.W = torch.empty(B, Lq - 1, Lq - 1, device=device, dtype=F32)
+
+    @staticmethod
+    def supported(Lq):
+        return bool(L.lib().cdll.wc_attn_mean_acc_supported(int(Lq)))
+
+    def add(self, qkv16, lse, B, Lq, H, DH):
+        if (B, Lq) != (self.B, self.Lq) or self.done >= self.n_layers:
+            raise RuntimeError(f"MapAccumulator: layer {self.done + 1} of {self.n_layers}, shape {(B, Lq)} != {(self.B, self.Lq)}")
+        L.lib().wc_attn_mean_acc(L.ptr(qkv16), L.ptr(lse), L.ptr(self.W), self.weight, 1 if self.done == 0 else 0, B, Lq, H, DH,
+                                 L.stream())
+        self.done += 1
+
+    def result(self):
+        if self.done != self.n_layers:
+            raise RuntimeError(f"MapAccumulator: {self.done} of {self.n_layers} layers were added")
+        return self.W
+
+
+def attention(qkv16, B, Lq, H, DH, want_mean=True, want_o32=False, acc=None):
     E = H * DH
     dev = qkv16.device
     lib = L.lib()
@@ -137,7 +161,9 @@
     o32 = torch.empty(B * Lq, E, device=dev, dtype=F32) if want_o32 else None
     lib.wc_attn_fwd(L.ptr(qkv16, F16, "qkv"), L.ptr(o16), L.ptr(o32), L.ptr(lse), B, Lq, H, DH, L.stream())
     mean = None
-    if want_mean:
+    if want_mean and acc is not None:
+        acc.add(qkv16, lse, B, Lq, H, DH)
+    elif want_mean:
         mean = torch.empty(B, Lq, Lq, device=dev, dtype=F32)
         lib.wc_attn_mean(L.ptr(qkv16), L.ptr(lse), L.ptr(mean), B, Lq, H, DH, L.stream())
     if want_o32:
```

Result: no change. 1363 images/sec (median of 6 runs) (+0.9%).
